# Immortal-ibr/Verifiable-Federated-Training-with-Zero-Knowledge-Proofs-ZK-FL-

Hardware: AMD Instinct MI355X
Metric: Groth16 proofs/sec (training-step circuit, ~2^18 constraints) at 1/8 MI355X (higher is better)
Workload: dtype u32; 1 GPU; groth16 prove, sgd_verified(128, 4, 7, 1000) (BATCH,DIM,DEPTH,PRECISION); constraints=261399, wires=262810, domain=262144, global_batch=20, step=20 proofs per GPU (one per slot), parallelism=replicas1, slots_in_flight=20, hw_queues=28

## Files before the change

### include/zkfl.h

```cpp
#ifndef ZKFL_H
#define ZKFL_H

#include <stddef.h>
#include <stdint.h>

#ifdef __cplusplus
extern "C" {
#endif

#define ZKFL_OK 0
#define ZKFL_E_ARG -1
#define ZKFL_E_FORMAT -2
#define ZKFL_E_PRIME -3
#define ZKFL_E_MISMATCH -4
#define ZKFL_E_DEVICE -5
#define ZKFL_E_OOM -6
#define ZKFL_E_CONSTRAINT -7
#define ZKFL_E_KEY -8

typedef struct zkfl_ctx zkfl_ctx;
typedef struct zkfl_key zkfl_key;
typedef struct zkfl_witness zkfl_witness;
typedef struct zkfl_wprog zkfl_wprog;
typedef struct zkfl_vkey zkfl_vkey;

int zkfl_version(void);
const char* zkfl_build_id(void);
const char* zkfl_last_error(void);
int zkfl_device_count(int* count);

int zkfl_ctx_create(int device, zkfl_ctx** out);
int zkfl_ctx_destroy(zkfl_ctx* ctx);
int zkfl_ctx_set_profiling(zkfl_ctx* ctx, int enabled);
int zkfl_ctx_profile(zkfl_ctx* ctx, const char* name, double* total_ms, uint64_t* launches, double* units,
                     double* median_ms);
int zkfl_ctx_profile_reset(zkfl_ctx* ctx);
int zkfl_ctx_synchronize(zkfl_ctx* ctx);

int zkfl_zkey_load(zkfl_ctx* ctx, const uint8_t* buf, size_t len, zkfl_key** out);
typedef struct zkfl_zkey_file zkfl_zkey_file;
int zkfl_zkey_file_open(const char* path, zkfl_zkey_file** out);
int zkfl_zkey_load_file(zkfl_ctx* ctx, const zkfl_zkey_file* f, zkfl_key** out);
int zkfl_zkey_file_close(zkfl_zkey_file* f);
int zkfl_key_free(zkfl_key* key);
int zkfl_key_info(const zkfl_key* key, uint32_t* n_vars, uint32_t* n_public, uint32_t* domain_size);
int zkfl_key_ab_shared(const zkfl_key* key, uint32_t* d_form, uint32_t* shared_wires, uint32_t* a_bases);
int zkfl_debug_ab_partition(const uint8_t* sec_a, const uint8_t* sec_b1, size_t n, uint32_t shard, uint32_t n_shards,
                            uint32_t* counts, uint32_t* sidx_out, uint8_t* img_out);
typedef struct zkfl_groups_info {
  uint32_t grouped;
  uint32_t learned;
  uint32_t groups;
  uint32_t non_rep;
  uint32_t bases[4];
  uint32_t bases_rep[4];
  uint32_t builds;
  uint32_t last_miss;
  double build_ms;
} zkfl_groups_info;
int zkfl_key_set_groups(zkfl_key* key, const uint32_t* rep, size_t n_vars);
int zkfl_key_learn_groups(zkfl_ctx* ctx, zkfl_key* key, const zkfl_witness* w);
int zkfl_key_groups(const zkfl_key* key, zkfl_groups_info* out);
int zkfl_debug_groups(const uint8_t* values, const uint8_t* sig, size_t n, uint32_t* rep_out, const uint32_t* sidx,
                      size_t n_bases, uint32_t u_base, uint32_t* sidx_out, uint32_t* start_out,
                      uint32_t* members_out);
int zkfl_key_set_slots(zkfl_key* key, int slots);

int zkfl_groth16_prove(zkfl_ctx* ctx, zkfl_key* key, const uint8_t* wtns, size_t wtns_len,
                       const uint8_t* rs, uint8_t proof_out[256], uint8_t* pub_out, size_t* npub);

int zkfl_witness_upload(zkfl_ctx* ctx, const zkfl_key* key, const uint8_t* wtns, size_t wtns_len,
                        zkfl_witness** out);
int zkfl_witness_free(zkfl_witness* w);
int zkfl_groth16_prove_resident(zkfl_ctx* ctx, zkfl_key* key, const zkfl_witness* w, const uint8_t* rs,
                                uint8_t proof_out[256]);
int zkfl_groth16_prove_batch(zkfl_ctx* ctx, zkfl_key* key, size_t n, const zkfl_witness* const* w,
                             const uint8_t* rs, uint8_t* proofs_out);

int zkfl_groth16_prove_multi(zkfl_ctx* ctx, size_t n, zkfl_key* const* keys, const zkfl_witness* const* w,
                             const uint8_t* rs, uint8_t* proofs_out);

int zkfl_zkey_load_shard(zkfl_ctx* ctx, const uint8_t* buf, size_t len, uint32_t shard, uint32_t n_shards,
                         zkfl_key** out);
int zkfl_key_shard(const zkfl_key* key, uint32_t* shard, uint32_t* n_shards);
int zkfl_groth16_prove_part_batch(zkfl_ctx* ctx, zkfl_key* key, size_t n, const zkfl_witness* const* w,
                                  const uint8_t* rs, uint8_t* parts_out);
int zkfl_groth16_assemble(zkfl_ctx* ctx, size_t n, size_t n_parts, const uint8_t* parts, const uint8_t* rs,
                          uint8_t* proofs_out);

int zkfl_debug_prove_parts(zkfl_ctx* ctx, zkfl_key* key, const uint8_t* wtns, size_t wtns_len, uint8_t* h_out,
                           uint8_t* msm_out);

int zkfl_debug_glv_split(const uint8_t k[32], uint8_t out[40]);

int zkfl_debug_g1_glv_mul(zkfl_ctx* ctx, size_t n, const uint8_t* points, const uint8_t* scalars, uint8_t* out);

int zkfl_debug_wtrace(zkfl_ctx* ctx, int op, uint32_t cap, void* out, uint32_t* count);

int zkfl_debug_ntt_coset(zkfl_ctx* ctx, uint8_t* data, uint32_t logn, uint32_t nvec, size_t vstride, int col_max);

int zkfl_msm_g1(zkfl_ctx* ctx, const uint8_t* bases, const uint8_t* scalars, size_t n, uint8_t out[64]);
int zkfl_msm_g2(zkfl_ctx* ctx, const uint8_t* bases, const uint8_t* scalars, size_t n, uint8_t out[128]);
int zkfl_ntt_coset(zkfl_ctx* ctx, uint8_t* data, uint32_t logn);

int zkfl_wprog_load(zkfl_ctx* ctx, const uint8_t* prog, size_t len, zkfl_wprog** out);
int zkfl_wprog_free(zkfl_wprog* prog);
int zkfl_wprog_info(const zkfl_wprog* prog, uint32_t* n_wires, uint32_t* n_inputs, uint32_t* n_public);
size_t zkfl_wtns_size(const zkfl_wprog* prog);
int zkfl_wprog_parse_inputs(const uint8_t* prog, size_t len, const char* input_json, uint8_t* inputs_out, size_t cap,
                            size_t* n_inputs);
int zkfl_witness_compute_json(zkfl_ctx* ctx, const zkfl_wprog* prog, const char* input_json, uint8_t* wtns_out);
int zkfl_witness_compute(zkfl_ctx* ctx, const zkfl_wprog* prog, size_t n, const uint8_t* inputs, uint8_t* wtns_out);
int zkfl_witness_compute_resident(zkfl_ctx* ctx, const zkfl_wprog* prog, const zkfl_key* key, size_t n,
                                  const uint8_t* inputs, zkfl_witness** out);

int zkfl_groth16_full_prove_batch(zkfl_ctx* ctx, zkfl_key* key, const zkfl_wprog* prog, size_t n,
                                  const uint8_t* inputs, const uint8_t* rs, uint8_t* proofs_out, uint8_t* pubs_out);

int zkfl_groth16_full_prove_json(zkfl_ctx* ctx, zkfl_key* key, const zkfl_wprog* prog, const char* input_json,
                                 const uint8_t* rs, uint8_t proof_out[256], uint8_t* pub_out);

int zkfl_groth16_full_prove_json_batch(zkfl_ctx* ctx, zkfl_key* key, const zkfl_wprog* prog, size_t n,
                                       const char* const* input_jsons, const uint8_t* rs, uint8_t* proofs_out,
                                       uint8_t* pubs_out);

int zkfl_groth16_full_prove_multi(zkfl_ctx* ctx, size_t n, zkfl_key* const* keys, const zkfl_wprog* const* progs,
                                  const uint8_t* const* inputs, const uint8_t* rs, uint8_t* proofs_out,
                                  uint8_t* const* pubs_out);

typedef struct zkfl_r1cs zkfl_r1cs;
typedef struct {
  uint32_t n_wires, n_pub_out, n_pub_in, n_prv_in, n_constraints;
  uint64_t n_labels, n_terms;
} zkfl_r1cs_header;
typedef struct {
  uint32_t n_failed, first;
  uint8_t a[32], b[32], c[32];
} zkfl_r1cs_report;
int zkfl_r1cs_parse(const uint8_t* buf, size_t len, zkfl_r1cs_header* out);
int zkfl_r1cs_load(zkfl_ctx* ctx, const uint8_t* buf, size_t len, zkfl_r1cs** out);
int zkfl_r1cs_info(const zkfl_r1cs* r1cs, zkfl_r1cs_header* out);
int zkfl_r1cs_free(zkfl_r1cs* r1cs);
int zkfl_r1cs_check(zkfl_ctx* ctx, const zkfl_r1cs* r1cs, size_t n, const uint8_t* const* wtns, const size_t* wtns_len,
                    zkfl_r1cs_report* reports);
int zkfl_r1cs_check_resident(zkfl_ctx* ctx, const zkfl_r1cs* r1cs, size_t n, const zkfl_witness* const* w,
                             zkfl_r1cs_report* reports);

#define ZKFL_KEYCHECK_HEADER 0
#define ZKFL_KEYCHECK_POINTS 1
#define ZKFL_KEYCHECK_COEFFICIENTS 2
#define ZKFL_KEYCHECK_A 3
#define ZKFL_KEYCHECK_B1 4
#define ZKFL_KEYCHECK_B2 5
#define ZKFL_KEYCHECK_IC 6
#define ZKFL_KEYCHECK_C 7
#define ZKFL_KEYCHECK_H 8
#define ZKFL_KEYCHECK_N 9
#define ZKFL_KEYCHECK_PASS 0
#define ZKFL_KEYCHECK_FAIL 1
#define ZKFL_KEYCHECK_NOT_RUN 2
typedef struct {
  uint32_t power;
  const uint8_t *L, *L2, *La, *Lb, *H0;
  size_t L_len, L2_len, La_len, Lb_len, H0_len;
  const uint8_t *alpha1, *beta1, *beta2;
} zkfl_ptau_view;
typedef struct {
  uint32_t status[ZKFL_KEYCHECK_N];
  uint32_t point_section, point_index, point_count;
  uint32_t coef_matrix, coef_row, coef_count;
} zkfl_zkey_report;
int zkfl_zkey_check(zkfl_ctx* ctx, const zkfl_r1cs* r1cs, const uint8_t* zkey, size_t zkey_len,
                    const zkfl_ptau_view* ptau, const uint8_t* rho, const uint8_t* sigma, zkfl_zkey_report* report);

int zkfl_groth16_verify(zkfl_ctx* ctx, const uint8_t* vk, size_t vk_len, const uint8_t* pub, size_t npub,
                        const uint8_t proof[256]);
int zkfl_groth16_verify_batch(zkfl_ctx* ctx, const uint8_t* vk, size_t vk_len, size_t n, const uint8_t* pubs,
                              size_t npub, const uint8_t* proofs, int32_t* results);
int zkfl_pairing(zkfl_ctx* ctx, size_t n, const uint8_t* g1, const uint8_t* g2, uint8_t* gt_out);
int zkfl_debug_miller_loop(zkfl_ctx* ctx, size_t n, const uint8_t* g1, const uint8_t* g2, uint8_t* out);

#define ZKFL_VERIFY_WAVE_MAX_PUBLIC 32
int zkfl_vkey_load(zkfl_ctx* ctx, const uint8_t* vk, size_t vk_len, zkfl_vkey** out);
int zkfl_vkey_info(const zkfl_vkey* key, uint32_t* n_public);
int zkfl_vkey_free(zkfl_vkey* key);

#define ZKFL_VERIFY_AUTO 0
#define ZKFL_VERIFY_LANES 1
#define ZKFL_VERIFY_WAVES 2
#define ZKFL_VERIFY_AUTO_WAVES_MAX 4096
int zkfl_groth16_verify_multi(zkfl_ctx* ctx, size_t n, const zkfl_vkey* const* vkeys, const uint8_t* const* pubs,
                              const size_t* npubs, const uint8_t* proofs, int32_t* results, int schedule);
typedef struct {
  uint32_t keys;
  uint32_t screened;
  uint32_t combined;
  uint32_t passed;
  uint32_t fallback;
} zkfl_round_report;
int zkfl_groth16_verify_round(zkfl_ctx* ctx, size_t n, const zkfl_vkey* const* vkeys, const uint8_t* const* pubs,
                              const size_t* npubs, const uint8_t* proofs, const uint8_t* z, int32_t* results,
                              zkfl_round_report* report);
int zkfl_debug_verify_round(zkfl_ctx* ctx, size_t n, const zkfl_vkey* const* vkeys, const uint8_t* const* pubs,
                            const size_t* npubs, const uint8_t* proofs, const uint8_t* z, size_t chunk,
                            uint8_t gt_out[384], int32_t* screened_out);
int zkfl_debug_wave_pairing(zkfl_ctx* ctx, size_t n, const uint8_t* g1, const uint8_t* g2, int final_exp,
                            uint8_t* out);

int zkfl_poseidon_params(uint32_t t, uint8_t* consts_out, uint8_t* xy_out, uint32_t* rp_out);
int zkfl_poseidon_batch(zkfl_ctx* ctx, uint32_t arity, size_t n, const uint8_t* inputs, uint8_t* out);
int zkfl_vector_hash_batch(zkfl_ctx* ctx, uint32_t len, size_t n, const uint8_t* values, uint8_t* out);
#define ZKFL_MERKLE_MAX_DEPTH 30
int zkfl_merkle_build(zkfl_ctx* ctx, const uint8_t* leaves, size_t n, uint32_t depth, uint8_t* tree_out);
int zkfl_dataset_commit(zkfl_ctx* ctx, const uint8_t* values, size_t n, uint32_t len, uint32_t depth,
                        uint8_t* tree_out);

int zkfl_setup_g1_gen_mul(zkfl_ctx* ctx, const uint8_t* scalars, size_t n, uint8_t* out);
int zkfl_setup_g2_gen_mul(zkfl_ctx* ctx, const uint8_t* scalars, size_t n, uint8_t* out);
// ... 15 lines not shown
```

### verifiable-federated-training-with-zero-knowledge-proofs-zk-fl-_amd/csrc/groups.h

```cpp
#pragma once
#include <stddef.h>
#include <stdint.h>
#include <string.h>

#include <algorithm>
#include <unordered_map>
#include <vector>

namespace zkfl {

inline bool groups_valid(const uint32_t* rep, size_t n) {
  for (size_t i = 0; i < n; i++)
    if (rep[i] > i || rep[rep[i]] != rep[i]) return false;
  return true;
}

inline void groups_learn(const uint32_t* w, size_t n, std::vector<uint32_t>& rep) {
  rep.resize(n);
  std::vector<uint32_t> big;
  for (size_t i = 0; i < n; i++) {
    rep[i] = (uint32_t)i;
    const uint32_t* v = w + 8 * i;
    if (v[4] | v[5] | v[6] | v[7]) big.push_back((uint32_t)i);
  }
  std::sort(big.begin(), big.end(), [&](uint32_t a, uint32_t b) {
    const int c = memcmp(w + 8 * (size_t)a, w + 8 * (size_t)b, 32);
    return c ? c < 0 : a < b;
  });
  for (size_t k = 1; k < big.size(); k++)
    if (memcmp(w + 8 * (size_t)big[k], w + 8 * (size_t)big[k - 1], 32) == 0) rep[big[k]] = rep[big[k - 1]];
}

inline void groups_refine(uint32_t* rep, const uint8_t* sig, size_t n) {
  std::unordered_map<uint64_t, uint32_t> first;
  for (size_t i = 0; i < n; i++) {
    const uint32_t r = rep[i];
    if ((sig[i] & ~sig[r]) == 0) continue;
    rep[i] = first.emplace((uint64_t)r << 8 | sig[i], (uint32_t)i).first->second;
  }
}

struct GroupQuery {
  std::vector<uint32_t> sidx;
  std::vector<uint32_t> start;
  std::vector<uint32_t> members;
  uint32_t groups = 0;
  uint32_t non_rep = 0;
};

inline void groups_query(const uint32_t* rep, uint32_t n_vars, const uint32_t* sidx, size_t n, uint32_t u_base,
                         GroupQuery& q) {
  constexpr uint32_t NONE = 0xFFFFFFFFu;
  std::vector<uint32_t> slot_of(n_vars, NONE), to(n, NONE);
  for (size_t j = 0; j < n; j++)
    if (sidx[j] < n_vars) slot_of[sidx[j]] = (uint32_t)j;
  q.sidx.assign(sidx, sidx + n);
  q.start.assign(n + 1, 0);
  q.groups = q.non_rep = 0;
  for (size_t j = 0; j < n; j++) {
    const uint32_t i = sidx[j];
    if (i >= n_vars || rep[i] == i || slot_of[rep[i]] == NONE) continue;
    to[j] = slot_of[rep[i]];
    q.sidx[j] = u_base + i;
    if (q.start[to[j] + 1]++ == 0) q.groups++;
    q.non_rep++;
  }
  for (size_t j = 0; j < n; j++) q.start[j + 1] += q.start[j];
  q.members.resize(q.non_rep);
  std::vector<uint32_t> cur(q.start.begin(), q.start.end() - 1);
  for (size_t j = 0; j < n; j++)
    if (to[j] != NONE) q.members[cur[to[j]]++] = (uint32_t)j;
}

}

#ifdef __HIPCC__
#include <hip/hip_runtime.h>

#include "curve.h"

namespace zkfl {

template <class F>
void group_sums(hipStream_t st, const Affine<F>* bases_w, int W, size_t n, const uint32_t* start,
                const uint32_t* members, Affine<F>* out);
void group_delta(hipStream_t st, const Fr* w, const uint32_t* rep, uint32_t n, Fr* u, uint32_t* cnt,
                 uint32_t* miss_out);

}
#endif
```

### verifiable-federated-training-with-zero-knowledge-proofs-zk-fl-_amd/csrc/groups.hip

```cpp
#include <hip/hip_runtime.h>
#include <stdint.h>

#include <chrono>
#include <cstdio>
#include <vector>

#include "devbufs.h"
#include "groups.h"
#include "objects.h"

using namespace zkfl;

namespace {

ZK_DEV Fq from_m29(const Fq& a) {
  Fq c = fp_zero<FqP>();
  c.v[7] = 0x08000000u;
  return fp_mul(a, c);
}

template <class F>
ZK_DEV Affine<F> load_base(const Affine<F>* __restrict__ p) {
  Affine<F> a = *p;
  Fq* q = reinterpret_cast<Fq*>(&a);
#pragma unroll
  for (int k = 0; k < (int)(sizeof(Affine<F>) / sizeof(Fq)); k++) q[k] = from_m29(q[k]);
  return a;
}

template <class F>
__global__ void __launch_bounds__(64) k_group_sums(const Affine<F>* __restrict__ bases_w, int W, size_t n,
                                                   const uint32_t* __restrict__ start,
                                                   const uint32_t* __restrict__ members, Affine<F>* __restrict__ out) {
  const size_t j = (size_t)blockIdx.x * blockDim.x + threadIdx.x;
  if (j >= n) return;
  const Affine<F> p = load_base<F>(bases_w + j * W);
  const uint32_t b = start[j], e = start[j + 1];
  if (b == e) {
    out[j] = p;
    return;
  }
  XYZZ<F> acc = xyzz_from_affine<F>(p);
  for (uint32_t m = b; m < e; m++) acc = xyzz_madd<F>(acc, load_base<F>(bases_w + (size_t)members[m] * W));
  out[j] = xyzz_to_affine<F>(acc);
}

constexpr int DELTA_T = 256;

__global__ void __launch_bounds__(DELTA_T) k_group_delta(const Fr* __restrict__ w, const uint32_t* __restrict__ rep,
                                                         uint32_t n, Fr* __restrict__ u, uint32_t* __restrict__ cnt,
                                                         uint32_t* __restrict__ miss_out) {
  ZK_LIGHT();
  const uint32_t i = blockIdx.x * DELTA_T + threadIdx.x;
  int nz = 0;
  if (i < n) {
    const uint32_t r = rep[i];
    Fr v = fp_zero<FrP>();
    if (r != i) {
      v = fp_sub(w[i], w[r]);
#pragma unroll
      for (int k = 0; k < 8; k++) nz |= v.v[k] != 0;
    }
    u[i] = v;
  }
  const int blk = __syncthreads_count(nz);
  if (threadIdx.x == 0) {
    if (blk) atomicAdd(&cnt[0], (uint32_t)blk);
    __threadfence();
    if (atomicAdd(&cnt[1], 1u) == gridDim.x - 1) {
      __threadfence();
      *miss_out = atomicExch(&cnt[0], 0u);
      cnt[1] = 0;
    }
  }
}

}

namespace zkfl {

template <class F>
void group_sums(hipStream_t st, const Affine<F>* bases_w, int W, size_t n, const uint32_t* start,
                const uint32_t* members, Affine<F>* out) {
  if (n) hipLaunchKernelGGL(k_group_sums<F>, dim3(zk_grid(n, 64)), dim3(64), 0, st, bases_w, W, n, start, members, out);
}
template void group_sums<FqOps>(hipStream_t, const G1Aff*, int, size_t, const uint32_t*, const uint32_t*, G1Aff*);
template void group_sums<Fq2Ops>(hipStream_t, const G2Aff*, int, size_t, const uint32_t*, const uint32_t*, G2Aff*);

void group_delta(hipStream_t st, const Fr* w, const uint32_t* rep, uint32_t n, Fr* u, uint32_t* cnt,
                 uint32_t* miss_out) {
  hipLaunchKernelGGL(k_group_delta, dim3(zk_grid(n, DELTA_T)), dim3(DELTA_T), 0, st, w, rep, n, u, cnt, miss_out);
}

void key_groups_release(zkfl_key* k) {
  msm_bases_free(k->gA);
  msm_bases_free(k->gB1);
  msm_bases_free(k->gB2);
  msm_bases_free(k->gCH);
  if (k->grp.d_rep) (void)hipFree(k->grp.d_rep);
  const uint32_t builds = k->grp.builds;
  k->grp = KeyGroups();
  k->grp.builds = builds;
}

}

namespace {

template <class F>
hipError_t build_query(const MsmBases<F>& plain, MsmBases<F>& out, const GroupQuery& q, uint32_t extra_start,
                       DevBufs& D, hipStream_t st) {
  ZK_CHECK(msm_bases_alloc(out, plain.n, plain.c));
  if (plain.n == 0) return hipSuccess;
  uint32_t *d_start, *d_members;
  Affine<F>* d_img;
  ZK_CHECK(D.get(&d_start, q.start.size()));
  ZK_CHECK(D.get(&d_members, q.members.size()));
  ZK_CHECK(D.get(&d_img, plain.n));
  ZK_CHECK(hipMemcpyAsync(d_start, q.start.data(), q.start.size() * 4, hipMemcpyHostToDevice, st));
  if (!q.members.empty())
    ZK_CHECK(hipMemcpyAsync(d_members, q.members.data(), q.members.size() * 4, hipMemcpyHostToDevice, st));
  group_sums<F>(st, plain.bases_w, msm_w_of(plain.c), plain.n, d_start, d_members, d_img);
  ZK_CHECK(hipGetLastError());
  return msm_bases_set(out, d_img, q.sidx.data(), extra_start, st, false);
}

int key_build_groups(zkfl_key* k, std::vector<uint32_t>& rep, bool learned, double host_ms) {
  const auto t0 = std::chrono::steady_clock::now();
  HIP_TRY(hipSetDevice(k->ctx->device), "hipSetDevice");
  int rc = key_reset_graphs(k);
  if (rc) return rc;
  key_groups_release(k);
  const uint32_t nV = k->nVars, X = nV, dom = k->n;
  std::vector<uint8_t> sig(nV, 0);
  for (int qi = 0; qi < 4; qi++)
    for (uint32_t i : k->q_sidx[qi])
      if (i < nV) sig[i] |= (uint8_t)(1u << qi);
  groups_refine(rep.data(), sig.data(), nV);
  const uint32_t u_base[4] = {X + 4, X + 4, X + 4, X + dom + 4};
  GroupQuery q[4];
  for (int qi = 0; qi < 4; qi++)
    groups_query(rep.data(), nV, k->q_sidx[qi].data(), k->q_sidx[qi].size(), u_base[qi], q[qi]);
  hipStream_t st = k->ctx->st;
  hipError_t e;
  {
    DevBufs D;
    e = hipMalloc(&k->grp.d_rep, (size_t)(nV ? nV : 1) * 4);
    if (e == hipSuccess) e = hipMemcpyAsync(k->grp.d_rep, rep.data(), (size_t)nV * 4, hipMemcpyHostToDevice, st);
    if (e == hipSuccess) e = build_query(k->bA, k->gA, q[0], X, D, st);
    if (e == hipSuccess) e = build_query(k->bB1, k->gB1, q[1], X, D, st);
    if (e == hipSuccess) e = build_query(k->bB2, k->gB2, q[2], X, D, st);
    if (e == hipSuccess) e = build_query(k->bCH, k->gCH, q[3], X, D, st);
    const hipError_t es = hipStreamSynchronize(st);
    if (e == hipSuccess) e = es;
  }
  if (e != hipSuccess) {
    key_groups_release(k);
    return hip_fail(e, "grouped base sets");
  }
  KeyGroups& g = k->grp;
  g.on = true;
  g.learned = learned;
  for (uint32_t i = 0; i < nV; i++) g.non_rep += rep[i] != i;
  std::vector<uint8_t> has(nV, 0);
  for (uint32_t i = 0; i < nV; i++)
    if (rep[i] != i && !has[rep[i]]) {
      has[rep[i]] = 1;
      g.groups++;
    }
  for (int qi = 0; qi < 4; qi++) {
    g.bases[qi] = (uint32_t)k->q_sidx[qi].size();
    g.bases_rep[qi] = g.bases[qi] - q[qi].non_rep;
  }
  g.builds++;
  g.build_ms = host_ms + std::chrono::duration<double, std::milli>(std::chrono::steady_clock::now() - t0).count();
  fprintf(stderr,
          "zkfl: key of %u wires: %u groups, %u non-representative wires; bases A %u -> %u, B %u -> %u, C+H %u -> %u; "
          "%s and built in %.1f ms\n",
          nV, g.groups, g.non_rep, g.bases[0], g.bases_rep[0], g.bases[1], g.bases_rep[1], g.bases[3], g.bases_rep[3],
          learned ? "learned" : "set", g.build_ms);
  return ZKFL_OK;
}

int groups_allowed(const zkfl_key* k) {
  if (k->nshards != 1) return fail(ZKFL_E_ARG, "groups: a sharded key keeps the plain form");
  if (!k->ctx->opts.groups) return fail(ZKFL_E_ARG, "groups: turned off on this context (ZKFL_GROUPS=0)");
  return ZKFL_OK;
}

}

int zkfl::key_learn_groups(zkfl_ctx* ctx, zkfl_key* k, const Fr* d_w) {
  const auto t0 = std::chrono::steady_clock::now();
  HIP_TRY(hipSetDevice(ctx->device), "hipSetDevice");
  std::vector<uint32_t> w((size_t)k->nVars * 8), rep;
  HIP_TRY(hipMemcpy(w.data(), d_w, w.size() * 4, hipMemcpyDeviceToHost), "download witness");
  groups_learn(w.data(), k->nVars, rep);
  const double ms = std::chrono::duration<double, std::milli>(std::chrono::steady_clock::now() - t0).count();
  return key_build_groups(k, rep, true, ms);
}

extern "C" {

int zkfl_key_set_groups(zkfl_key* key, const uint32_t* rep, size_t n_vars) {
  if (!key) return fail(ZKFL_E_ARG, "null key");
  if (!rep) {
    HIP_TRY(hipSetDevice(key->ctx->device), "hipSetDevice");
    const int rc = key_reset_graphs(key);
    if (rc) return rc;
    key_groups_release(key);
    return ZKFL_OK;
  }
  int rc = groups_allowed(key);
  if (rc) return rc;
  if (n_vars != key->nVars) return fail(ZKFL_E_ARG, "groups: rep must hold one entry per wire of the key");
  if (!groups_valid(rep, n_vars)) return fail(ZKFL_E_ARG, "groups: rep[i] <= i and rep[rep[i]] == rep[i] must hold");
  std::vector<uint32_t> r(rep, rep + n_vars);
  return key_build_groups(key, r, false, 0.0);
}

int zkfl_key_learn_groups(zkfl_ctx* ctx, zkfl_key* key, const zkfl_witness* w) {
  if (!ctx || !key || !w) return fail(ZKFL_E_ARG, "null argument");
  if (key->ctx != ctx) return fail(ZKFL_E_ARG, "groups: key of another context");
  if (w->key != key) return fail(ZKFL_E_MISMATCH, "witness uploaded for another key");
  const int rc = groups_allowed(key);
  if (rc) return rc;
  return key_learn_groups(ctx, key, w->d);
}

int zkfl_key_groups(const zkfl_key* key, zkfl_groups_info* out) {
  if (!key || !out) return fail(ZKFL_E_ARG, "null argument");
  const KeyGroups& g = key->grp;
  *out = zkfl_groups_info();
  out->grouped = g.on;
  out->learned = g.learned;
  out->groups = g.groups;
  out->non_rep = g.non_rep;
  for (int i = 0; i < 4; i++) {
    out->bases[i] = g.on ? g.bases[i] : (uint32_t)key->q_sidx[i].size();
    out->bases_rep[i] = g.on ? g.bases_rep[i] : out->bases[i];
  }
  out->builds = g.builds;
  out->last_miss = g.last_miss;
  out->build_ms = g.build_ms;
  return ZKFL_OK;
}

int zkfl_debug_groups(const uint8_t* values, const uint8_t* sig, size_t n, uint32_t* rep_out, const uint32_t* sidx,
                      size_t n_bases, uint32_t u_base, uint32_t* sidx_out, uint32_t* start_out,
                      uint32_t* members_out) {
  if (!rep_out || n > 0x7FFFFFF0u || (n_bases && !sidx)) return fail(ZKFL_E_ARG, "debug_groups: bad arguments");
  std::vector<uint32_t> rep;
  if (values) {
    std::vector<uint32_t> w(n * 8);
    memcpy(w.data(), values, n * 32);
    groups_learn(w.data(), n, rep);
  } else {
    rep.assign(rep_out, rep_out + n);
    if (!groups_valid(rep.data(), n)) return fail(ZKFL_E_ARG, "debug_groups: not a partition");
  }
  if (sig) groups_refine(rep.data(), sig, n);
  memcpy(rep_out, rep.data(), n * 4);
  if (sidx_out || start_out || members_out) {
    GroupQuery q;
    groups_query(rep.data(), (uint32_t)n, sidx, n_bases, u_base, q);
    if (sidx_out) memcpy(sidx_out, q.sidx.data(), n_bases * 4);
    if (start_out) memcpy(start_out, q.start.data(), (n_bases + 1) * 4);
    if (members_out && !q.members.empty()) memcpy(members_out, q.members.data(), q.members.size() * 4);
  }
  return ZKFL_OK;
}

}
```

### verifiable-federated-training-with-zero-knowledge-proofs-zk-fl-_amd/csrc/objects.h

```cpp
#pragma once
#include <hip/hip_runtime.h>
#include <stdint.h>

#include <atomic>
#include <string>
#include <vector>

#include "curve.h"
#include "field.h"
#include "msm_api.h"
#include "ntt.h"
#include "prof.h"
#include "wtrace.h"
#include "zkfl.h"

namespace zkfl {
struct VkDev;
struct PosTables;
struct WProg;

int fail(int code, const std::string& msg);
int hip_fail(hipError_t e, const char* where);
}

#define HIP_TRY(x, where)                              \
  do {                                                 \
    hipError_t _e = (x);                               \
    if (_e != hipSuccess) return ::zkfl::hip_fail(_e, where); \
  } while (0)

using namespace zkfl;

struct WitPipe;

struct SchedOpts {
  bool graph = true;
  bool stagger = true;
  bool lowlat = true;
  bool fast_wsum = true;
  int small_logn = 16;
  bool ab_shared = true;
  bool groups = true;
  int group_min_batch = 8;
};

struct zkfl_ctx {
  int device = 0;
  hipStream_t st = nullptr;
  SchedOpts opts;
  Profiler prof;
  zkfl::VkDev* vk = nullptr;
  zkfl::PosTables* pos = nullptr;
  void* asm_buf = nullptr;
  size_t asm_cap = 0;
  WtBuf wt;
  std::atomic<int> refs{1};
};

struct ProofSlot {
  hipStream_t st_main = nullptr;
  hipEvent_t ev_done = nullptr;
  MsmScratch<FqOps> g1s;
#if ZK_KNOCKOUT & 2
  MsmScratch<FqOps> g1s_ko[3];
#endif
  MsmTail<FqOps> g1t[4];
  MsmScratch<Fq2Ops> g2s;
  MsmTail<Fq2Ops> g2t;
  Fr* extra = nullptr;
  Fr* abc = nullptr;
  Fr* abc_head = nullptr;
  Fr* abc_tail = nullptr;
  Fr* h = nullptr;
  uint32_t* grp_cnt = nullptr;
  zkfl_key* key = nullptr;
  bool grouped_run = false;
  G1P* res = nullptr;
  G2P* resB2 = nullptr;
  Fr* d_rs = nullptr;
  uint32_t* d_parts = nullptr;
  uint8_t* pinned = nullptr;
  hipStream_t st_lat[2] = {nullptr, nullptr};
  hipEvent_t ev_lat[3] = {nullptr, nullptr, nullptr};
  MsmScratch<FqOps> g1s_b;
  MsmScratch<FqOps> g1s_a;
  hipGraph_t graph = nullptr;
  hipGraphExec_t graph_exec = nullptr;
  Fr* w_stage = nullptr;
  uint32_t direct_proofs = 0;
  bool nnz_alias = false;
  bool busy = false;
  int index = 0;
  size_t job = 0;
  uint8_t* out_proof = nullptr;
  uint8_t* out_part = nullptr;
};

struct KeyGroups {
  bool on = false;
  bool learned = false;
  uint32_t groups = 0;
  uint32_t non_rep = 0;
  uint32_t bases[4] = {0, 0, 0, 0};
  uint32_t bases_rep[4] = {0, 0, 0, 0};
  double build_ms = 0;
  uint32_t builds = 0;
  uint32_t last_miss = 0;
  uint32_t* d_rep = nullptr;
};

struct zkfl_key {
  zkfl_ctx* ctx = nullptr;
  uint32_t nVars = 0, nPub = 0, n = 0;
  int logn = 0;
  size_t nC = 0;
  size_t K = 0;
  uint32_t* rows = nullptr;
  uint32_t* cols = nullptr;
  Fr* coefs = nullptr;
  uint32_t cshift = 0;
  MsmBases<FqOps> bA, bB1;
  MsmBases<Fq2Ops> bB2;
  MsmBases<FqOps> bCH;
  MsmBases<FqOps> gA, gB1, gCH;
  MsmBases<Fq2Ops> gB2;
  KeyGroups grp;
  std::vector<uint32_t> q_sidx[4];
  Fr* dbg_zero = nullptr;
  bool a_diff = false;
  uint32_t ab_shared = 0;
  bool share_b = false;
  bool front = false;
  int msm_c = MSM_C;
  NttPlan ntt;
  std::vector<ProofSlot*> slots;
  int max_slots = 3;
  uint32_t shard = 0, nshards = 1;
  WitPipe* wpipe = nullptr;
};

struct zkfl_witness {
  const zkfl_key* key = nullptr;
  Fr* d = nullptr;
  std::vector<uint8_t> pub;
};

struct zkfl_wprog {
  zkfl_ctx* ctx = nullptr;
  zkfl::WProg* p = nullptr;
};

struct zkfl_vkey {
  zkfl_ctx* ctx = nullptr;
  zkfl::VkDev* vk = nullptr;
  void* wtab = nullptr;
  bool wave_ok = false;
};

namespace zkfl {
void ctx_retain(zkfl_ctx* ctx);
void ctx_release(zkfl_ctx* ctx);
int get_slot(zkfl_key* k, size_t idx, ProofSlot** out);
void key_release_slots(zkfl_key* k);
int key_reset_graphs(zkfl_key* k);
void key_groups_release(zkfl_key* k);
int key_learn_groups(zkfl_ctx* ctx, zkfl_key* k, const Fr* d_w);
constexpr size_t MISS_OFF = 456;
}
```

### verifiable-federated-training-with-zero-knowledge-proofs-zk-fl-_amd/csrc/poly.h

```cpp
#pragma once
#include <hip/hip_runtime.h>
#include <stdint.h>

#include "field.h"
#include "glv.h"

namespace zkfl {

constexpr uint32_t ABC_L = 16;

struct AbcTerms {
  const uint32_t* cols;
  const Fr* coefs;
  uint32_t cshift;
};

struct ProofStart {
  uint4* buckets[5];
  uint32_t nvec[5];
  uint32_t* nnz[5];
  uint32_t* live[5];
  int n;
  const uint64_t* w_src_host;
  uint4* w_dst;
  uint32_t w_nvec;
};

constexpr int RS_WORDS = (64 + 4 * (int)sizeof(GlvScalar)) / 4;

__device__ __forceinline__ Fr abc_row(const uint32_t* __restrict__ rp, uint32_t r, uint32_t K,
                                      const Fr* __restrict__ head, const Fr* __restrict__ tail,
                                      const Fr* __restrict__ abc) {
  const uint32_t s = rp[r], e = rp[r + 1];
  if (s == e) return fp_zero<FrP>();
  const uint32_t c0 = s / ABC_L, c1 = (e - 1) / ABC_L;
  const bool starts = (s == c0 * ABC_L);
  if (c0 == c1) {
    const uint32_t cend = (c0 + 1) * ABC_L < K ? (c0 + 1) * ABC_L : K;
    if (starts) return head[c0];
    if (e == cend) return tail[c0];
    return abc[r];
  }
  Fr acc = starts ? head[c0] : tail[c0];
  for (uint32_t c = c0 + 1; c <= c1; c++) acc = fp_add(acc, head[c]);
  return acc;
}

void abc_chunks(hipStream_t st, const uint32_t* rp, uint32_t nrows, const AbcTerms& T, const Fr* w, uint32_t K,
                Fr* head, Fr* tail, Fr* abc);
void abc_rows(hipStream_t st, const uint32_t* rp, size_t n, uint32_t K, const Fr* head, const Fr* tail, Fr* abc);
void join_h(hipStream_t st, const Fr* abc, size_t n, Fr* h);
void proof_start(hipStream_t st, const uint32_t* rs_host, uint32_t* d_rs, Fr* extra, int plain, uint32_t* res3,
                 const ProofStart& ps);
void fr_std_to_mont(hipStream_t st, Fr* a, size_t n);
void fr_mont_to_std(hipStream_t st, Fr* a, size_t n);

}
```

### verifiable-federated-training-with-zero-knowledge-proofs-zk-fl-_amd/csrc/poly.hip

```cpp
#include "poly.h"

#include "common.h"
#include "msm_api.h"
#include "wtrace.h"

using namespace zkfl;

namespace {

template <bool PACKED>
__global__ void __launch_bounds__(64) k_abc_chunks(const uint32_t* __restrict__ rp, uint32_t nrows, AbcTerms T,
                                                   const Fr* __restrict__ w, uint32_t K, Fr* __restrict__ head,
                                                   Fr* __restrict__ tail, Fr* __restrict__ abc) {
  ZK_WT(WT_ABC);
  ZK_LIGHT();
  const uint32_t c = blockIdx.x * blockDim.x + threadIdx.x;
  const uint32_t p0 = c * ABC_L;
  if (p0 >= K) return;
  const uint32_t p1 = p0 + ABC_L < K ? p0 + ABC_L : K;
  const uint32_t* __restrict__ cols = T.cols;
  const Fr* __restrict__ coefs = T.coefs;
  const uint32_t cmask = PACKED ? (1u << T.cshift) - 1u : 0xFFFFFFFFu;
  auto coef_of = [&](uint32_t t, uint32_t p) { return PACKED ? coefs[t >> T.cshift] : coefs[p]; };
  auto row_of = [&](uint32_t p, uint32_t lo) {
    uint32_t hi = nrows - 1;
    while (lo < hi) {
      const uint32_t mid = (lo + hi + 1) >> 1;
      if (rp[mid] <= p) lo = mid;
      else hi = mid - 1;
    }
    return lo;
  };
  uint32_t r = row_of(p0, 0), rend = rp[r + 1];
  Fr acc = fp_zero<FrP>();
  bool first = true;
  uint32_t t1 = (p0 + 1 < p1) ? cols[p0 + 1] : 0u;
  const uint32_t t0 = cols[p0];
  Fr wv = w[t0 & cmask], cf = coef_of(t0, p0);
  for (uint32_t p = p0; p < p1; p++) {
    Fr wn, cn;
    uint32_t t2 = 0;
    if (p + 1 < p1) {
      wn = w[t1 & cmask];
      cn = coef_of(t1, p + 1);
    }
    if (p + 2 < p1) t2 = cols[p + 2];
    if (p == rend) {
      if (first) head[c] = acc;
      else abc[r] = acc;
      first = false;
      acc = fp_zero<FrP>();
      r++;
      rend = rp[r + 1];
      if (rend == p) {
        r = row_of(p, r);
        rend = rp[r + 1];
      }
    }
    acc = fp_add(acc, fp_mul(cf, wv));
    wv = wn;
    cf = cn;
    t1 = t2;
  }
  if (first) head[c] = acc;
  else tail[c] = acc;
}

__global__ void __launch_bounds__(256) k_abc_rows(const uint32_t* __restrict__ rp, size_t n, uint32_t K,
                                                  const Fr* __restrict__ head, const Fr* __restrict__ tail,
                                                  Fr* __restrict__ abc) {
  ZK_WT(WT_ABC_ROWS);
  ZK_LIGHT();
  const size_t j = (size_t)blockIdx.x * blockDim.x + threadIdx.x;
  if (j >= n) return;
  const Fr a = abc_row(rp, (uint32_t)j, K, head, tail, abc);
  const Fr b = abc_row(rp, (uint32_t)(n + j), K, head, tail, abc);
  abc[j] = a;
  abc[n + j] = b;
  abc[2 * n + j] = fp_mul(a, b);
}

__global__ void k_join(const Fr* __restrict__ abc, size_t n, Fr* __restrict__ h) {
  ZK_WT(WT_JOIN);
  ZK_LIGHT();
  size_t j = (size_t)blockIdx.x * blockDim.x + threadIdx.x;
  if (j >= n) return;
#if ZK_KNOCKOUT & 4
  Fr v = fp_add(fp_mul(abc[j], abc[n + j]), abc[2 * n + j]);
#else
  Fr v = fp_sub(fp_mul(abc[j], abc[n + j]), abc[2 * n + j]);
#endif
  h[j] = fp_from_mont(v);
}

__global__ void __launch_bounds__(256) k_proof_start(const uint32_t* __restrict__ rs_host, uint32_t* __restrict__ d_rs,
                                                     Fr* __restrict__ extra, int plain, uint32_t* __restrict__ res3,
                                                     const ProofStart ps) {
  ZK_WT(WT_SET_EXTRA);
  ZK_LIGHT();
  const int y = blockIdx.y;
  if (ps.w_dst) {
    __shared__ const uint4* src;
    if (threadIdx.x == 0) src = reinterpret_cast<const uint4*>(*ps.w_src_host);
    __syncthreads();
    const size_t nb = (size_t)gridDim.x * gridDim.y * blockDim.x;
    for (size_t i = ((size_t)y * gridDim.x + blockIdx.x) * blockDim.x + threadIdx.x; i < ps.w_nvec; i += nb)
      ps.w_dst[i] = src[i];
  }
  if (y == 0 && blockIdx.x == 2 && threadIdx.x < RS_WORDS) d_rs[threadIdx.x] = rs_host[threadIdx.x];
  if (y == 0 && blockIdx.x == 0 && threadIdx.x == 0) {
    const Fr* rs = reinterpret_cast<const Fr*>(rs_host);
    Fr one = fp_zero<FrP>();
    one.v[0] = plain ? 0u : 1u;
    Fr r = plain ? fp_zero<FrP>() : rs[0];
    Fr s = plain ? fp_zero<FrP>() : rs[1];
    extra[0] = one;
    extra[1] = r;
    extra[2] = s;
    extra[3] = fp_from_mont(fp_neg(fp_mul(fp_to_mont(r), fp_to_mont(s))));
  }
  if (y == 0 && blockIdx.x == 1 && res3 && threadIdx.x < sizeof(G1P) / 4) res3[threadIdx.x] = 0u;
  if (y >= ps.n) return;
  uint4* b = ps.buckets[y];
  const size_t nv = ps.nvec[y];
  for (size_t i = (size_t)blockIdx.x * blockDim.x + threadIdx.x; i < nv; i += (size_t)gridDim.x * blockDim.x)
    b[i] = make_uint4(0, 0, 0, 0);
  if (blockIdx.x == 0 && threadIdx.x == 0) *ps.nnz[y] = 0;
  if (blockIdx.x == 0 && threadIdx.x < MSM_LIVE_LEVELS) ps.live[y][threadIdx.x] = 0;
}

__global__ void k_fr_std_to_mont(Fr* __restrict__ a, size_t n) {
  size_t i = (size_t)blockIdx.x * blockDim.x + threadIdx.x;
  if (i >= n) return;
  a[i] = fp_to_mont(a[i]);
}

__global__ void k_fr_mont_to_std(Fr* __restrict__ a, size_t n) {
  size_t i = (size_t)blockIdx.x * blockDim.x + threadIdx.x;
  if (i >= n) return;
  a[i] = fp_from_mont(a[i]);
}

}

namespace zkfl {

hipError_t zk_wtrace_bind_poly(const WtBuf& b) { return zk_wtrace_bind_tu(b); }

void abc_chunks(hipStream_t st, const uint32_t* rp, uint32_t nrows, const AbcTerms& T, const Fr* w, uint32_t K,
                Fr* head, Fr* tail, Fr* abc) {
  if (T.cshift)
    hipLaunchKernelGGL(k_abc_chunks<true>, dim3(zk_grid((K + ABC_L - 1) / ABC_L, 64)), dim3(64), 0, st, rp, nrows, T, w,
                       K, head, tail, abc);
  else
    hipLaunchKernelGGL(k_abc_chunks<false>, dim3(zk_grid((K + ABC_L - 1) / ABC_L, 64)), dim3(64), 0, st, rp, nrows, T, w,
                       K, head, tail, abc);
}

void abc_rows(hipStream_t st, const uint32_t* rp, size_t n, uint32_t K, const Fr* head, const Fr* tail, Fr* abc) {
  hipLaunchKernelGGL(k_abc_rows, dim3(zk_grid(n, 256)), dim3(256), 0, st, rp, n, K, head, tail, abc);
}

void join_h(hipStream_t st, const Fr* abc, size_t n, Fr* h) {
  hipLaunchKernelGGL(k_join, dim3(zk_grid(n, 256)), dim3(256), 0, st, abc, n, h);
}

void proof_start(hipStream_t st, const uint32_t* rs_host, uint32_t* d_rs, Fr* extra, int plain, uint32_t* res3,
                 const ProofStart& ps) {
  hipLaunchKernelGGL(k_proof_start, dim3(128, ps.n), dim3(256), 0, st, rs_host, d_rs, extra, plain, res3, ps);
}

void fr_std_to_mont(hipStream_t st, Fr* a, size_t n) {
  hipLaunchKernelGGL(k_fr_std_to_mont, dim3(zk_grid(n, 256)), dim3(256), 0, st, a, n);
}

void fr_mont_to_std(hipStream_t st, Fr* a, size_t n) {
  hipLaunchKernelGGL(k_fr_mont_to_std, dim3(zk_grid(n, 256)), dim3(256), 0, st, a, n);
}

}
```

### verifiable-federated-training-with-zero-knowledge-proofs-zk-fl-_amd/csrc/prove.hip

```cpp
#include <hip/hip_runtime.h>
#include <stdint.h>
#include <string.h>
#include <sys/random.h>

#include <algorithm>
#include <atomic>
#include <chrono>
#include <condition_variable>
#include <mutex>
#include <string>
#include <thread>
#include <vector>

#include "assemble.h"
#include "glv.h"
#include "groups.h"
#include "host_parse.h"
#include "objects.h"
#include "poly.h"
#include "witness.h"

using namespace zkfl;

namespace {

constexpr size_t W_PTR_OFF = 448;

inline uint32_t* proof_out(ProofSlot* s) { return reinterpret_cast<uint32_t*>(s->pinned); }

void slot_drop_lowlat(ProofSlot* s) {
  for (hipStream_t& st : s->st_lat)
    if (st) {
      (void)hipStreamSynchronize(st);
      (void)hipStreamDestroy(st);
      st = nullptr;
    }
  for (hipEvent_t& e : s->ev_lat)
    if (e) {
      (void)hipEventDestroy(e);
      e = nullptr;
    }
}

void slot_release(ProofSlot* s) {
  if (!s) return;
  if (s->st_main) (void)hipStreamSynchronize(s->st_main);
  slot_drop_lowlat(s);
  if (s->nnz_alias) s->g2t.nnz = nullptr;
  msm_scratch_free(s->g1s);
#if ZK_KNOCKOUT & 2
  for (MsmScratch<FqOps>& x : s->g1s_ko) msm_scratch_free(x);
#endif
  for (auto& t : s->g1t) msm_tail_free(t);
  msm_scratch_free(s->g2s);
  msm_tail_free(s->g2t);
  void* ptrs[] = {s->abc, s->abc_head, s->abc_tail, s->h, s->res, s->resB2, s->d_rs, s->d_parts,
                  s->w_stage, s->grp_cnt};
  for (void* p : ptrs)
    if (p) (void)hipFree(p);
  if (s->pinned) (void)hipHostFree(s->pinned);
  msm_scratch_free(s->g1s_b);
  msm_scratch_free(s->g1s_a);
  if (s->graph_exec) (void)hipGraphExecDestroy(s->graph_exec);
  if (s->graph) (void)hipGraphDestroy(s->graph);
  if (s->ev_done) (void)hipEventDestroy(s->ev_done);
  if (s->st_main) (void)hipStreamDestroy(s->st_main);
  delete s;
}

hipError_t slot_side_resources(ProofSlot* s, const zkfl_key* k, bool need_streams) {
  if (need_streams) {
    for (hipStream_t& st : s->st_lat)
      if (!st) ZK_CHECK(hipStreamCreateWithFlags(&st, hipStreamNonBlocking));
    for (hipEvent_t& e : s->ev_lat)
      if (!e) ZK_CHECK(hipEventCreateWithFlags(&e, hipEventDisableTiming));
  }
  if (!s->g1s_a.keys_out) ZK_CHECK(msm_scratch_alloc(s->g1s_a, k->bA.n, k->msm_c, k->ctx->st));
  if (!s->g1s_b.keys_out) ZK_CHECK(msm_scratch_alloc(s->g1s_b, k->bB1.n, k->msm_c, k->ctx->st));
  return hipSuccess;
}

hipError_t slot_create(zkfl_key* k, ProofSlot** out) {
  ProofSlot* s = new ProofSlot();
  *out = s;
  const size_t nV = k->nVars, n = k->n;
  const size_t cap1 = std::max<size_t>({k->bA.n, k->bB1.n, k->bCH.n});
  hipStream_t st = k->ctx->st;
  ZK_CHECK(hipStreamCreateWithFlags(&s->st_main, hipStreamNonBlocking));
  ZK_CHECK(hipEventCreateWithFlags(&s->ev_done, hipEventDisableTiming));
  const int c = k->msm_c;
  ZK_CHECK(msm_scratch_alloc(s->g1s, cap1, c, st));
#if ZK_KNOCKOUT & 2
  for (MsmScratch<FqOps>& x : s->g1s_ko) {
    ZK_CHECK(msm_scratch_alloc(x, cap1, c, st));
    ZK_CHECK(hipMemsetAsync(x.keys_out, 0, cap1 * msm_w_of(c) * sizeof(uint16_t), st));
    ZK_CHECK(hipMemsetAsync(x.vals_out, 0, cap1 * msm_w_of(c) * sizeof(uint32_t), st));
  }
#endif
  const size_t caps[4] = {k->bA.n, k->bB1.n, k->bCH.n, k->bCH.n};
  for (int i = 0; i < 4; i++) ZK_CHECK(msm_tail_alloc(s->g1t[i], caps[i], c));
  ZK_CHECK(msm_scratch_alloc(s->g2s, k->bB2.n, c, st));
  ZK_CHECK(msm_tail_alloc(s->g2t, k->bB2.n, c));
  if (k->share_b && !ZK_KNOCKOUT) {
    ZK_CHECK(hipFree(s->g2t.nnz));
    s->g2t.nnz = s->g1t[1].nnz;
    s->nnz_alias = true;
  }
  if (k->ctx->opts.graph) ZK_CHECK(hipMalloc(&s->w_stage, nV * 32));
  if (k->front) ZK_CHECK(slot_side_resources(s, k, false));
  const bool may_group = k->ctx->opts.groups && k->nshards == 1;
  ZK_CHECK(hipMalloc(&s->h, (n + 4 + (may_group ? nV : 0)) * 32));
  s->extra = s->h + n;
  ZK_CHECK(hipMalloc(&s->grp_cnt, 2 * sizeof(uint32_t)));
  ZK_CHECK(hipMemsetAsync(s->grp_cnt, 0, 2 * sizeof(uint32_t), st));
  s->key = k;
  ZK_CHECK(hipMalloc(&s->abc, n * 3 * 32));
  const size_t abc_chunks = (k->K + ABC_L - 1) / ABC_L + 1;
  ZK_CHECK(hipMalloc(&s->abc_head, abc_chunks * 32));
  ZK_CHECK(hipMalloc(&s->abc_tail, abc_chunks * 32));
  ZK_CHECK(hipMalloc(&s->res, 5 * sizeof(G1P)));
  ZK_CHECK(hipMalloc(&s->resB2, sizeof(G2P)));
  ZK_CHECK(hipMalloc(&s->d_rs, 2 * 32 + 4 * sizeof(GlvScalar)));
  ZK_CHECK(hipMalloc(&s->d_parts, PART_WORDS * 4));
  ZK_CHECK(hipHostMalloc(&s->pinned, 2048, hipHostMallocCoherent));
  return hipStreamSynchronize(st);
}

}

int zkfl::get_slot(zkfl_key* k, size_t idx, ProofSlot** out) {
  size_t want = idx % (size_t)k->max_slots;
  while (k->slots.size() <= want) {
    ProofSlot* s = nullptr;
    hipError_t e = slot_create(k, &s);
    if (e != hipSuccess) {
      slot_release(s);
      return hip_fail(e, "proof slot allocation");
    }
    s->index = (int)k->slots.size();
    k->slots.push_back(s);
  }
  *out = k->slots[want];
  return ZKFL_OK;
}

constexpr int WIT_SETS = 4;
struct WitPipe {
  struct Set {
    Fr* W = nullptr;
    Fr* d = nullptr;
    uint32_t* in = nullptr;
    uint32_t* fail = nullptr;
    Fr** outs = nullptr;
    uint8_t* pin_in = nullptr;
    hipEvent_t ev = nullptr;
  };
  size_t G = 0, nw = 0, n_in = 0;
  hipStream_t st = nullptr;
  Set set[WIT_SETS];
};

namespace {

void wpipe_release(WitPipe* p) {
  if (!p) return;
  if (p->st) (void)hipStreamSynchronize(p->st);
  for (auto& b : p->set) {
    for (void* q : {(void*)b.W, (void*)b.d, (void*)b.in, (void*)b.fail, (void*)b.outs})
      if (q) (void)hipFree(q);
    if (b.pin_in) (void)hipHostFree(b.pin_in);
    if (b.ev) (void)hipEventDestroy(b.ev);
  }
  if (p->st) (void)hipStreamDestroy(p->st);
  delete p;
}

}

int zkfl::key_reset_graphs(zkfl_key* k) {
  for (ProofSlot* s : k->slots)
    if (s->busy) return fail(ZKFL_E_ARG, "slots busy");
  for (ProofSlot* s : k->slots) {
    if (s->st_main) (void)hipStreamSynchronize(s->st_main);
    if (s->graph_exec) (void)hipGraphExecDestroy(s->graph_exec);
    if (s->graph) (void)hipGraphDestroy(s->graph);
    s->graph_exec = nullptr;
    s->graph = nullptr;
  }
  return ZKFL_OK;
}

void zkfl::key_release_slots(zkfl_key* k) {
  wpipe_release(k->wpipe);
  k->wpipe = nullptr;
  for (ProofSlot* s : k->slots) slot_release(s);
  k->slots.clear();
}

namespace {

hipError_t wpipe_get(zkfl_key* k, size_t G, size_t nw, size_t n_in, WitPipe** out) {
  WitPipe* p = k->wpipe;
  if (p && p->G == G && p->nw == nw && p->n_in == n_in) {
    *out = p;
    return hipSuccess;
  }
  wpipe_release(p);
  k->wpipe = p = new WitPipe();
  p->G = G;
  p->nw = nw;
  p->n_in = n_in;
  ZK_CHECK(hipStreamCreateWithFlags(&p->st, hipStreamNonBlocking));
  for (auto& b : p->set) {
    ZK_CHECK(hipMalloc(&b.W, G * nw * 32));
    ZK_CHECK(hipMalloc(&b.d, G * nw * 32));
    ZK_CHECK(hipMalloc(&b.in, G * n_in * 32 + 16));
    ZK_CHECK(hipMalloc(&b.fail, G * 4));
    ZK_CHECK(hipMalloc(&b.outs, G * sizeof(Fr*)));
    ZK_CHECK(hipHostMalloc(&b.pin_in, G * n_in * 32 + 16));
    ZK_CHECK(hipEventCreateWithFlags(&b.ev, hipEventDisableTiming));
    std::vector<Fr*> ptrs(G);
    for (size_t j = 0; j < G; j++) ptrs[j] = b.d + j * nw;
    ZK_CHECK(hipMemcpy(b.outs, ptrs.data(), G * sizeof(Fr*), hipMemcpyHostToDevice));
  }
  *out = p;
  return hipSuccess;
}

int get_rs(const uint8_t* rs, uint32_t out[16]) {
  if (rs) {
    memcpy(out, rs, 64);
    if (!fr_lt_r(out) || !fr_lt_r(out + 8)) return fail(ZKFL_E_ARG, "r/s must be < r");
    return ZKFL_OK;
  }
  for (int k = 0; k < 2; k++) {
    for (int tries = 0;; tries++) {
      uint8_t b[32];
      if (getrandom(b, 32, 0) != 32) return fail(ZKFL_E_DEVICE, "getrandom failed");
      b[31] &= 0x3f;
      memcpy(out + 8 * k, b, 32);
      if (fr_lt_r(out + 8 * k)) break;
      if (tries > 64) return fail(ZKFL_E_DEVICE, "rng");
    }
  }
  return ZKFL_OK;
}

enum class ProofMode {
  Proof,
  Parts,
  SplitPart,
};

enum class Schedule { Lowlat, Front, Chain };

struct ProofPlan {
  ProofMode mode;
  Schedule schedule;
  bool share_b_sort;
  bool light_first;
  bool joint_tails;
  bool fast_wsum;
  bool graph;
  bool grouped;
};

struct PlanBases {
  const MsmBases<FqOps>&A, &B1, &CH;
  const MsmBases<Fq2Ops>& B2;
};
inline PlanBases plan_bases(const zkfl_key* k, const ProofPlan& p) {
  if (p.grouped) return {k->gA, k->gB1, k->gCH, k->gB2};
  return {k->bA, k->bB1, k->bCH, k->bB2};
}

ProofPlan plan_proof(const SchedOpts& o, const zkfl_key* k, const ProofSlot* s, ProofMode mode, bool batch_of_one,
                     const Profiler* prof) {
  ProofPlan p = {};
  p.mode = mode;
  p.grouped = mode == ProofMode::Proof && k->grp.on && !ZK_KNOCKOUT;
  const bool plain = mode == ProofMode::Proof && k->share_b && !prof->serialize && !ZK_KNOCKOUT;
  const bool want_lowlat = batch_of_one && o.lowlat;
  p.graph = o.graph && s->w_stage && !want_lowlat && plain && !prof->on && s->direct_proofs > 0;
  p.share_b_sort = k->share_b && !(ZK_KNOCKOUT & 32);
  if (want_lowlat && plain) {
    p.schedule = Schedule::Lowlat;
    p.fast_wsum = o.fast_wsum;
    return p;
  }
  p.joint_tails = p.share_b_sort && k->front;
  const bool front = p.joint_tails && mode != ProofMode::Parts && !(ZK_KNOCKOUT & 2);
  p.schedule = front ? Schedule::Front : Schedule::Chain;
  p.light_first = !front && o.stagger && (s->index & 1) && !prof->serialize;
  p.fast_wsum = o.fast_wsum && k->logn <= o.small_logn;
  return p;
}

inline const GlvScalar* glv_halves(const ProofSlot* s) {
  return reinterpret_cast<const GlvScalar*>(reinterpret_cast<const uint8_t*>(s->d_rs) + 64);
}

void start(zkfl_key* k, ProofSlot* s, const ProofPlan& p) {
  const bool parts = p.mode == ProofMode::Parts;
  const int ntails = parts ? 4 : 3;
  ProofStart ps = {};
  auto add = [&](void* buckets, size_t bytes, uint32_t* nnz, uint32_t* live) {
    ps.buckets[ps.n] = static_cast<uint4*>(buckets);
    ps.nvec[ps.n] = (uint32_t)(bytes / sizeof(uint4));
    ps.nnz[ps.n] = nnz;
    ps.live[ps.n] = live;
    ps.n++;
  };
  const size_t nb = msm_nb_of(k->msm_c);
  for (int i = 0; i < ntails; i++) add(s->g1t[i].buckets, nb * sizeof(G1P), s->g1t[i].nnz, s->g1t[i].live);
  if (p.share_b_sort) add(s->g2t.buckets, nb * sizeof(G2P), s->g2t.nnz, s->g2t.live);
  uint32_t* res3 = parts ? nullptr : reinterpret_cast<uint32_t*>(s->res + 3);
  if (p.graph) {
    ps.w_src_host = reinterpret_cast<const uint64_t*>(s->pinned + W_PTR_OFF);
    ps.w_dst = reinterpret_cast<uint4*>(s->w_stage);
    ps.w_nvec = (uint32_t)((size_t)k->nVars * 32 / sizeof(uint4));
  }
  proof_start(s->st_main, reinterpret_cast<const uint32_t*>(s->pinned + 256), reinterpret_cast<uint32_t*>(s->d_rs),
              s->extra, parts, res3, ps);
}

hipError_t abc_ntt(zkfl_key* k, ProofSlot* s, const Fr* d_w, hipStream_t st, Profiler* prof) {
  const size_t n = k->n;
  int pi = prof->begin("abc", st);
  if (k->K) {
    const uint32_t K = (uint32_t)k->K;
    const AbcTerms T = {k->cols, k->coefs, k->cshift};
    abc_chunks(st, k->rows, (uint32_t)(2 * n), T, d_w, K, s->abc_head, s->abc_tail, s->abc);
  }
  abc_rows(st, k->rows, n, (uint32_t)k->K, s->abc_head, s->abc_tail, s->abc);
  prof->end(pi, st, (double)k->K);
  pi = prof->begin("ntt", st);
  if (!(ZK_KNOCKOUT & 4)) ZK_CHECK(ntt_coset_shift(k->ntt, s->abc, 3, n, st));
  prof->end(pi, st, 3.0 * (double)n);
  join_h(st, s->abc, n, s->h);
  return hipSuccess;
}

hipError_t b2_from_b1_sort(const MsmBases<Fq2Ops>& bB2, ProofSlot* s, const MsmScratch<FqOps>& sorted, hipStream_t st,
                           Profiler* prof) {
  if (!s->nnz_alias)
    ZK_CHECK(hipMemcpyAsync(s->g2t.nnz, s->g1t[1].nnz, sizeof(uint32_t), hipMemcpyDeviceToDevice, st));
  return msm_accumulate_sorted(bB2, sorted.keys_out, sorted.vals_out, s->g2t, st, prof, "msm_accumulate_g2");
}

int finish(const zkfl_key* k, ProofSlot* s, const ProofPlan& p, Profiler* prof) {
  hipStream_t st = s->st_main;
  if (k->a_diff) fold_a(st, s->res);
  if (p.mode == ProofMode::SplitPart) {
    part_out(st, s->res, s->resB2, s->d_parts);
    HIP_TRY(hipMemcpyAsync(s->pinned + 512, s->d_parts, PART_WORDS * 4, hipMemcpyDeviceToHost, st), "download part");
  }
  if (p.mode == ProofMode::Proof && !(ZK_KNOCKOUT & 1)) {
    const int pa = prof->begin("assemble", st);
    assemble(st, 1, s->res, s->resB2, glv_halves(s), proof_out(s));
    prof->end(pa, st, 1.0);
  }
  return ZKFL_OK;
}

int run_lowlat(zkfl_key* k, ProofSlot* s, const Fr* d_w, const ProofPlan& p, Profiler* prof) {
  HIP_TRY(slot_side_resources(s, k, true), "latency schedule resources");
  hipStream_t st = s->st_main, sb = s->st_lat[0], sa = s->st_lat[1];
  hipEvent_t ev = s->ev_lat[0], ev_b2 = s->ev_lat[1], ev_t = s->ev_lat[2];
  const uint32_t *W = (const uint32_t*)d_w, *E = (const uint32_t*)s->extra;
  const PlanBases b = plan_bases(k, p);
  MsmTail<FqOps>* tails[3] = {&s->g1t[0], &s->g1t[1], &s->g1t[2]};
  G1P* outs[3] = {s->res + 0, s->res + 1, s->res + 2};
  MsmTail<Fq2Ops>* t2 = &s->g2t;
  G2P* o2 = s->resB2;
  HIP_TRY(hipEventRecord(ev, st), "event");
  HIP_TRY(hipStreamWaitEvent(sb, ev, 0), "wait");
  HIP_TRY(msm_sort(b.B1, s->g1s_b, s->g1t[1].nnz, W, E, sb), "msm B sort");
  HIP_TRY(hipEventRecord(ev, sb), "event");
  HIP_TRY(hipStreamWaitEvent(sa, ev, 0), "wait");
  HIP_TRY(b2_from_b1_sort(b.B2, s, s->g1s_b, sb, prof), "msm B2");
  HIP_TRY(msm_tails(&t2, &o2, 1, sb, p.fast_wsum), "msm B2 tail");
  HIP_TRY(hipEventRecord(ev_b2, sb), "event");
  HIP_TRY(msm_accumulate_sorted(b.B1, s->g1s_b.keys_out, s->g1s_b.vals_out, s->g1t[1], sa, prof,
                                   "msm_accumulate_g1"), "msm B1");
  HIP_TRY(msm_accumulate(b.A, s->g1s_a, s->g1t[0], W, E, sa, prof, "msm_accumulate_g1"), "msm A");
  HIP_TRY(msm_tails(tails, outs, 2, sa, p.fast_wsum), "msm tails A, B1");
  if (k->a_diff) fold_a(sa, s->res);
  assemble_t(sa, s->res, glv_halves(s), proof_out(s));
  HIP_TRY(hipEventRecord(ev_t, sa), "event");
  HIP_TRY(abc_ntt(k, s, d_w, st, prof), "ntt");
  HIP_TRY(msm_accumulate(b.CH, s->g1s, s->g1t[2], W, (const uint32_t*)s->h, st, prof, "msm_accumulate_g1"),
          "msm C+H");
  HIP_TRY(msm_tails(&tails[2], &outs[2], 1, st, p.fast_wsum), "msm tail C+H");
  HIP_TRY(hipStreamWaitEvent(st, ev_b2, 0), "wait");
  HIP_TRY(hipStreamWaitEvent(st, ev_t, 0), "wait");
  const int pa = prof->begin("assemble", st);
  assemble_c(st, s->res, s->resB2, proof_out(s));
  prof->end(pa, st, 1.0);
  return ZKFL_OK;
}

int run_front(zkfl_key* k, ProofSlot* s, const Fr* d_w, const ProofPlan& p, Profiler* prof) {
  hipStream_t st = s->st_main;
  const uint32_t *W = (const uint32_t*)d_w, *E = (const uint32_t*)s->extra;
  HIP_TRY(abc_ntt(k, s, d_w, st, prof), "ntt");
  const PlanBases b = plan_bases(k, p);
  const MsmBases<FqOps>* bs[3] = {&b.A, &b.B1, &b.CH};
  MsmScratch<FqOps>* ss[3] = {&s->g1s_a, &s->g1s_b, &s->g1s};
  MsmTail<FqOps>* tails[3] = {&s->g1t[0], &s->g1t[1], &s->g1t[2]};
  uint32_t* nn[3] = {s->g1t[0].nnz, s->g1t[1].nnz, s->g1t[2].nnz};
  const uint32_t* sc[3] = {W, W, W};
  const uint32_t* ex[3] = {E, E, (const uint32_t*)s->h};
  HIP_TRY(msm_sort_multi(bs, ss, nn, sc, ex, 3, st), "msm A, B1, C+H sorts");
  const uint16_t* kk[3] = {ss[0]->keys_out, ss[1]->keys_out, ss[2]->keys_out};
  const uint32_t* vv[3] = {ss[0]->vals_out, ss[1]->vals_out, ss[2]->vals_out};
  HIP_TRY(msm_accumulate_sorted_multi(bs, kk, vv, tails, 3, st), "msm A, B1, C+H");
  HIP_TRY(b2_from_b1_sort(b.B2, s, s->g1s_b, st, prof), "msm B2");
  G1P* outs[3] = {s->res + 0, s->res + 1, s->res + 2};
  MsmTail<Fq2Ops>* t2 = &s->g2t;
  G2P* o2 = s->resB2;
  HIP_TRY(msm_tails_joint(tails, outs, 3, &t2, &o2, 1, st, p.fast_wsum), "msm tails (G1 + G2)");
  return finish(k, s, p, prof);
}

int run_chain(zkfl_key* k, ProofSlot* s, const Fr* d_w, const ProofPlan& p, Profiler* prof) {
  hipStream_t st = s->st_main;
  const bool parts = p.mode == ProofMode::Parts;
  if (parts && !k->dbg_zero) return fail(ZKFL_E_ARG, "parity hook: zeros not allocated");
  const uint32_t *W = (const uint32_t*)d_w, *E = (const uint32_t*)s->extra, *H = (const uint32_t*)s->h,
                 *Z = (const uint32_t*)k->dbg_zero;
#if ZK_KNOCKOUT & 2
  MsmScratch<FqOps>&sA = s->g1s_ko[0], &sB = s->g1s_ko[1], &sCH = s->g1s_ko[2];
#else
  MsmScratch<FqOps>&sA = s->g1s, &sB = s->g1s, &sCH = s->g1s;
#endif
  const PlanBases b = plan_bases(k, p);
  MsmTail<FqOps>* tails[4] = {&s->g1t[0], &s->g1t[1], &s->g1t[2], &s->g1t[3]};
  G1P* outs[4] = {s->res + 0, s->res + 1, s->res + 2, s->res + 3};
  MsmTail<Fq2Ops>* t2 = &s->g2t;
  G2P* o2 = s->resB2;
  if (!p.share_b_sort && !(ZK_KNOCKOUT & 32))
    HIP_TRY(msm_run(b.B2, s->g2s, s->g2t, W, E, s->resB2, st, prof, "msm_accumulate_g2"), "msm B2");
  if (p.light_first) HIP_TRY(abc_ntt(k, s, d_w, st, prof), "ntt");
  HIP_TRY(msm_accumulate(b.A, sA, s->g1t[0], W, E, st, prof, "msm_accumulate_g1"), "msm A");
  if (p.share_b_sort) {
    HIP_TRY(msm_sort(b.B1, sB, s->g1t[1].nnz, W, E, st), "msm B1 sort");
    HIP_TRY(msm_accumulate_sorted(b.B1, sB.keys_out, sB.vals_out, s->g1t[1], st, prof, "msm_accumulate_g1"),
            "msm B1");
    HIP_TRY(b2_from_b1_sort(b.B2, s, sB, st, prof), "msm B2");
    if (!p.joint_tails) HIP_TRY(msm_tails(&t2, &o2, 1, st, p.fast_wsum), "msm B2 tail");
  } else {
    HIP_TRY(msm_accumulate(b.B1, sB, s->g1t[1], W, E, st, prof, "msm_accumulate_g1"), "msm B1");
  }
  if (parts) HIP_TRY(msm_accumulate(b.CH, s->g1s, s->g1t[2], W, Z, st, prof, "msm_accumulate_g1"), "msm C");
  if (!p.light_first) HIP_TRY(abc_ntt(k, s, d_w, st, prof), "ntt");
  if (parts)
    HIP_TRY(msm_accumulate(b.CH, s->g1s, s->g1t[3], Z, H, st, prof, "msm_accumulate_g1"), "msm H");
  else
    HIP_TRY(msm_accumulate(b.CH, sCH, s->g1t[2], W, H, st, prof, "msm_accumulate_g1"), "msm C+H");
  const int ntails = parts ? 4 : 3;
  if (p.joint_tails)
    HIP_TRY(msm_tails_joint(tails, outs, ntails, &t2, &o2, 1, st, p.fast_wsum), "msm tails (G1 + G2)");
  else
    HIP_TRY(msm_tails(tails, outs, ntails, st, p.fast_wsum), "msm tails");
  return finish(k, s, p, prof);
}

int run_proof(zkfl_ctx* ctx, zkfl_key* k, ProofSlot* s, const Fr* d_w, const ProofPlan& p) {
  Profiler* prof = &ctx->prof;
  const int pp = prof->begin("prove", s->st_main);
  start(k, s, p);
  if (p.grouped)
    group_delta(s->st_main, d_w, k->grp.d_rep, k->nVars, s->extra + 4, s->grp_cnt,
                reinterpret_cast<uint32_t*>(s->pinned + MISS_OFF));
  const int rc = p.schedule == Schedule::Lowlat  ? run_lowlat(k, s, d_w, p, prof)
                 : p.schedule == Schedule::Front ? run_front(k, s, d_w, p, prof)
                                                 : run_chain(k, s, d_w, p, prof);
  if (rc) return rc;
  prof->end(pp, s->st_main, 1.0);
  return ZKFL_OK;
}

int enqueue_proof_graph(zkfl_ctx* ctx, zkfl_key* k, ProofSlot* s, const ProofPlan& p) {
  hipStream_t st = s->st_main;
  if (!s->graph_exec) {
    HIP_TRY(hipStreamBeginCapture(st, hipStreamCaptureModeThreadLocal), "begin capture");
    const int rc = run_proof(ctx, k, s, s->w_stage, p);
    hipError_t e = hipStreamEndCapture(st, &s->graph);
    if (rc == ZKFL_OK && e == hipSuccess) e = hipGraphInstantiate(&s->graph_exec, s->graph, nullptr, nullptr, 0);
    if (rc || e != hipSuccess) {
      if (s->graph) (void)hipGraphDestroy(s->graph);
      s->graph = nullptr;
      s->graph_exec = nullptr;
      return rc ? rc : hip_fail(e, "graph capture");
    }
  }
  HIP_TRY(hipGraphLaunch(s->graph_exec, st), "graph launch");
  return ZKFL_OK;
}

int enqueue_proof(zkfl_ctx* ctx, zkfl_key* k, ProofSlot* s, const Fr* d_w, const uint32_t rs_host[16], ProofMode mode,
                  bool batch_of_one) {
  memcpy(s->pinned + 256, rs_host, 64);
  GlvScalar* ks = reinterpret_cast<GlvScalar*>(s->pinned + 320);
  glv_split(rs_host + 8, ks[0], ks[1]);
  glv_split(rs_host, ks[2], ks[3]);
  const ProofPlan p = plan_proof(ctx->opts, k, s, mode, batch_of_one, &ctx->prof);
  s->grouped_run = p.grouped;
  int rc;
  if (p.graph) {
    const uint64_t src = reinterpret_cast<uint64_t>(d_w);
    memcpy(s->pinned + W_PTR_OFF, &src, sizeof(src));
    rc = enqueue_proof_graph(ctx, k, s, p);
  } else {
    s->direct_proofs++;
    rc = run_proof(ctx, k, s, d_w, p);
  }
  if (rc) return rc;
  HIP_TRY(hipEventRecord(s->ev_done, s->st_main), "event");
  HIP_TRY(hipGetLastError(), "launch");
  return ZKFL_OK;
}

constexpr int WAIT_US = 50;
static hipError_t host_wait(hipEvent_t ev, bool poll) {
  if (!poll) return hipEventSynchronize(ev);
  for (;;) {
    const hipError_t e = hipEventQuery(ev);
    if (e != hipErrorNotReady) return e;
    std::this_thread::sleep_for(std::chrono::microseconds(WAIT_US));
  }
}

int wait_slot(ProofSlot* s, bool poll = false) {
  HIP_TRY(host_wait(s->ev_done, poll), "sync");
  if (s->out_proof) memcpy(s->out_proof, s->pinned, 256);
  if (s->out_part) memcpy(s->out_part, s->pinned + 512, PART_WORDS * 4);
  if (s->grouped_run) memcpy(&s->key->grp.last_miss, s->pinned + MISS_OFF, 4);
  s->grouped_run = false;
  s->busy = false;
  return ZKFL_OK;
}

struct Job {
  zkfl_key* key = nullptr;
  const Fr* w = nullptr;
  hipEvent_t w_ready = nullptr;
  const uint8_t* rs = nullptr;
  uint8_t* proof_out = nullptr;
  uint8_t* part_out = nullptr;
};

int learn_for_batch(zkfl_ctx* ctx, const Job& J, size_t n) {
  zkfl_key* k = J.key;
  if (!ctx->opts.groups || ZK_KNOCKOUT || n < (size_t)ctx->opts.group_min_batch || k->nshards != 1 || J.part_out)
    return ZKFL_OK;
  const KeyGroups& g = k->grp;
  if (g.on && !(g.learned && 2 * (uint64_t)g.last_miss > g.non_rep)) return ZKFL_OK;
  if (J.w_ready) HIP_TRY(hipEventSynchronize(J.w_ready), "wait for the witness group");
  return key_learn_groups(ctx, k, J.w);
}

template <class GetJob>
int run_jobs(zkfl_ctx* ctx, size_t n, GetJob job) {
  HIP_TRY(hipSetDevice(ctx->device), "hipSetDevice");
  struct PerKey {
    zkfl_key* key;
    size_t issued = 0;
  };
  std::vector<PerKey> cursor;
  auto issue = [&](PerKey& pk, size_t i, const Job& J, const uint32_t* rsl) -> int {
    ProofSlot* s = nullptr;
    int rc = get_slot(J.key, pk.issued++, &s);
    if (rc) return rc;
    if (s->busy) {
      rc = wait_slot(s, n > 1);
      if (rc) return rc;
    }
    s->job = i;
    s->out_proof = J.part_out ? nullptr : J.proof_out;
    s->out_part = J.part_out;
    if (J.w_ready) {
      hipError_t e = hipStreamWaitEvent(s->st_main, J.w_ready, 0);
      if (e != hipSuccess) return hip_fail(e, "wait for the witness group");
    }
    rc = enqueue_proof(ctx, J.key, s, J.w, rsl, J.part_out ? ProofMode::SplitPart : ProofMode::Proof, n == 1);
    if (rc) return rc;
    s->busy = true;
    return ZKFL_OK;
  };
  int rc = ZKFL_OK;
  for (size_t i = 0; i < n && rc == ZKFL_OK; i++) {
    Job J;
    rc = job(i, J);
    if (rc) break;
    if (J.key->nshards != 1 && !J.part_out) {
      rc = fail(ZKFL_E_ARG, "this key is shard " + std::to_string(J.key->shard) + " of " +
                                std::to_string(J.key->nshards) +
                                " of a split proof: prove parts (zkfl_groth16_prove_part_batch) and assemble them");
      break;
    }
    uint32_t rsl[16];
    rc = get_rs(J.rs, rsl);
    if (rc) break;
    size_t c = 0;
    while (c < cursor.size() && cursor[c].key != J.key) c++;
    if (c == cursor.size()) {
      cursor.emplace_back();
      cursor.back().key = J.key;
      rc = learn_for_batch(ctx, J, n);
      if (rc) break;
    }
    rc = issue(cursor[c], i, J, rsl);
  }
  for (auto& pk : cursor) {
    for (ProofSlot* s : pk.key->slots)
      if (s->busy) {
        int r2 = wait_slot(s, n > 1);
        if (rc == ZKFL_OK) rc = r2;
      }
  }
  return rc;
}

}

extern "C" {

int zkfl_groth16_prove_resident(zkfl_ctx* ctx, zkfl_key* key, const zkfl_witness* w, const uint8_t* rs,
                                uint8_t proof_out[256]) {
  return zkfl_groth16_prove_batch(ctx, key, 1, &w, rs, proof_out);
}

int zkfl_key_set_slots(zkfl_key* key, int slots) {
  if (!key || slots < 1 || slots > 32) return fail(ZKFL_E_ARG, "slots must be in 1..32");
  (void)hipSetDevice(key->ctx->device);
  for (ProofSlot* s : key->slots) {
    if (s->busy) return fail(ZKFL_E_ARG, "slots busy");
  }
  while ((int)key->slots.size() > slots) {
    slot_release(key->slots.back());
    key->slots.pop_back();
  }
  if (slots > 1)
    for (ProofSlot* s : key->slots) slot_drop_lowlat(s);
  key->max_slots = slots;
  return ZKFL_OK;
}

int zkfl_groth16_prove_batch(zkfl_ctx* ctx, zkfl_key* key, size_t n, const zkfl_witness* const* w,
                             const uint8_t* rs, uint8_t* proofs_out) {
  if (!ctx || !key || (!w && n) || (!proofs_out && n)) return fail(ZKFL_E_ARG, "null argument");
  for (size_t i = 0; i < n; i++) {
    if (!w[i] || w[i]->key != key) return fail(ZKFL_E_MISMATCH, "witness uploaded for another key");
  }
  return run_jobs(ctx, n, [&](size_t i, Job& J) {
    J.key = key;
    J.w = w[i]->d;
    J.rs = rs ? rs + 64 * i : nullptr;
    J.proof_out = proofs_out + 256 * i;
    return ZKFL_OK;
  });
}

int zkfl_groth16_prove_part_batch(zkfl_ctx* ctx, zkfl_key* key, size_t n, const zkfl_witness* const* w,
                                  const uint8_t* rs, uint8_t* parts_out) {
  if (!ctx || !key || (n && (!w || !rs || !parts_out))) return fail(ZKFL_E_ARG, "prove_part: null argument");
  for (size_t i = 0; i < n; i++) {
    if (!w[i] || w[i]->key != key) return fail(ZKFL_E_MISMATCH, "witness uploaded for another key");
  }
  return run_jobs(ctx, n, [&](size_t i, Job& J) {
    J.key = key;
    J.w = w[i]->d;
    J.rs = rs + 64 * i;
    J.part_out = parts_out + PART_WORDS * 4 * i;
    return ZKFL_OK;
  });
}

int zkfl_groth16_assemble(zkfl_ctx* ctx, size_t n, size_t n_parts, const uint8_t* parts, const uint8_t* rs,
                          uint8_t* proofs_out) {
  if (!ctx || (n && (!parts || !rs || !proofs_out)) || n_parts < 1 || n_parts > 1024)
    return fail(ZKFL_E_ARG, "assemble: bad arguments");
  if (n == 0) return ZKFL_OK;
  for (size_t i = 0; i < n * n_parts * (PART_WORDS / 8); i++)
    if (!fq_lt_q(reinterpret_cast<const uint32_t*>(parts + 32 * i)))
      return fail(ZKFL_E_ARG, "assemble: part coordinate " + std::to_string(i) + " is not < q");
  std::vector<uint8_t> ks(n * 4 * sizeof(GlvScalar));
  for (size_t i = 0; i < n; i++) {
    uint32_t rsl[16];
    int rc = get_rs(rs + 64 * i, rsl);
// ... 235 lines not shown
    }
    cv.notify_all();
    for (auto& t : th) t.join();
  }
  void work() {
    for (;;) {
      const size_t i = next.fetch_add(1);
      if (i >= n) return;
      {
        std::unique_lock<std::mutex> g(mu);
        cv.wait(g, [&] { return stop || i < consumed + AHEAD; });
        if (stop) return;
      }
      std::vector<uint32_t> v;
      std::string e;
      int r = texts[i] ? wprog_inputs_json(prog, texts[i], v, e) : ZKFL_E_ARG;
      if (!texts[i]) e = "null input json";
      if (r == ZKFL_OK && v.size() != n_in * 8) {
        r = ZKFL_E_ARG;
        e = "input json does not fill the program's inputs";
      }
      v.resize(n_in * 8 + 8);
      {
        std::lock_guard<std::mutex> g(mu);
        vec[i] = std::move(v);
        err[i] = std::move(e);
        rc[i] = r;
        done[i] = 1;
      }
      cv.notify_all();
    }
  }
  int get(size_t i, const uint8_t** out) {
    std::unique_lock<std::mutex> g(mu);
    if (i > 0) std::vector<uint32_t>().swap(vec[i - 1]);
    consumed = i;
    cv.notify_all();
    cv.wait(g, [&] { return done[i] != 0; });
    if (rc[i]) return fail(rc[i], "input " + std::to_string(i) + ": " + err[i]);
    *out = reinterpret_cast<const uint8_t*>(vec[i].data());
    return ZKFL_OK;
  }
};
}

int zkfl_groth16_full_prove_json_batch(zkfl_ctx* ctx, zkfl_key* key, const zkfl_wprog* prog, size_t n,
                                       const char* const* input_jsons, const uint8_t* rs, uint8_t* proofs_out,
                                       uint8_t* pubs_out) {
  if (!ctx || (n && (!input_jsons || !proofs_out))) return fail(ZKFL_E_ARG, "full_prove_json_batch: null argument");
  size_t n_in = 0;
  int rc = full_prove_check(ctx, key, prog, 0, nullptr, &n_in);
  if (rc || n == 0) return rc;
  JsonParsePool pool(prog->p, input_jsons, n, n_in);
  return full_prove_piped(
      ctx, n, [&](size_t) { return key; }, [&](size_t) { return (const WProg*)prog->p; },
      [&](size_t i, const uint8_t** in) { return pool.get(i, in); }, rs, proofs_out,
      [&](size_t i) { return pubs_out ? pubs_out + (size_t)key->nPub * 32 * i : nullptr; });
}

int zkfl_groth16_full_prove_multi(zkfl_ctx* ctx, size_t n, zkfl_key* const* keys, const zkfl_wprog* const* progs,
                                  const uint8_t* const* inputs, const uint8_t* rs, uint8_t* proofs_out,
                                  uint8_t* const* pubs_out) {
  if (!ctx || (n && (!keys || !progs || !inputs || !proofs_out))) return fail(ZKFL_E_ARG, "full_prove_multi: null argument");
  std::vector<size_t> n_in(n);
  for (size_t i = 0; i < n; i++) {
    int rc = full_prove_check(ctx, keys[i], progs[i], 1, inputs[i], &n_in[i]);
    if (rc) return fail(rc, "job " + std::to_string(i) + ": " + zkfl_last_error());
  }
  std::vector<std::pair<const zkfl_key*, const zkfl_wprog*>> kp;
  for (size_t i = 0; i < n; i++) {
    size_t c = 0;
    while (c < kp.size() && kp[c].first != keys[i]) c++;
    if (c == kp.size()) kp.push_back({keys[i], progs[i]});
    else if (kp[c].second != progs[i])
      return fail(ZKFL_E_ARG, "full_prove_multi: job " + std::to_string(i) +
                                  " uses its key with another witness program than an earlier job");
  }
  return full_prove_piped(
      ctx, n, [&](size_t i) { return keys[i]; }, [&](size_t i) { return (const WProg*)progs[i]->p; },
      [&](size_t i, const uint8_t** in) {
        *in = inputs[i];
        return ZKFL_OK;
      },
      rs, proofs_out, [&](size_t i) { return pubs_out ? pubs_out[i] : nullptr; });
}

int zkfl_groth16_prove(zkfl_ctx* ctx, zkfl_key* key, const uint8_t* wtns, size_t wtns_len, const uint8_t* rs,
                       uint8_t proof_out[256], uint8_t* pub_out, size_t* npub) {
  zkfl_witness* w = nullptr;
  int rc = zkfl_witness_upload(ctx, key, wtns, wtns_len, &w);
  if (rc) return rc;
  rc = zkfl_groth16_prove_resident(ctx, key, w, rs, proof_out);
  if (rc == ZKFL_OK) {
    if (pub_out) memcpy(pub_out, w->pub.data(), w->pub.size());
    if (npub) *npub = key->nPub;
  }
  zkfl_witness_free(w);
  return rc;
}

int zkfl_debug_prove_parts(zkfl_ctx* ctx, zkfl_key* key, const uint8_t* wtns, size_t wtns_len, uint8_t* h_out,
                           uint8_t* msm_out) {
  zkfl_witness* w = nullptr;
  int rc = zkfl_witness_upload(ctx, key, wtns, wtns_len, &w);
  if (rc) return rc;
  ProofSlot* s = nullptr;
  rc = get_slot(key, 0, &s);
  uint32_t zeros[16] = {0};
  if (rc == ZKFL_OK && !key->dbg_zero) {
    const size_t bytes = std::max<size_t>(key->nVars, (size_t)key->n + 4) * 32;
    hipError_t e = hipMalloc(&key->dbg_zero, bytes);
    if (e == hipSuccess) e = hipMemsetAsync(key->dbg_zero, 0, bytes, s->st_main);
    if (e == hipSuccess) e = hipStreamSynchronize(s->st_main);
    if (e != hipSuccess) rc = hip_fail(e, "parity hook zeros");
  }
  if (rc == ZKFL_OK && s->busy) rc = wait_slot(s);
  if (rc == ZKFL_OK) {
    s->out_proof = nullptr;
    s->out_part = nullptr;
    rc = enqueue_proof(ctx, key, s, w->d, zeros, ProofMode::Parts, false);
  }
  if (rc == ZKFL_OK) rc = wait_slot(s);
  hipStream_t st = s ? s->st_main : ctx->st;
  uint32_t* d_o = nullptr;
  if (rc == ZKFL_OK && msm_out) {
    hipError_t e = hipMalloc(&d_o, 64 * 4 + 128);
    if (e == hipSuccess) {
      point_out(st, s->res, 4, d_o);
      point_out(st, s->resB2, 1, d_o + 64);
      e = hipGetLastError();
    }
    std::vector<uint8_t> tmp(64 * 4 + 128);
    if (e == hipSuccess) e = hipMemcpyAsync(tmp.data(), d_o, tmp.size(), hipMemcpyDeviceToHost, st);
    if (e == hipSuccess) e = hipStreamSynchronize(st);
    if (e != hipSuccess) rc = hip_fail(e, "debug parts");
    if (rc == ZKFL_OK) {
      memcpy(msm_out, tmp.data(), 64);
      memcpy(msm_out + 64, tmp.data() + 64, 64);
      memcpy(msm_out + 128, tmp.data() + 256, 128);
      memcpy(msm_out + 256, tmp.data() + 128, 64);
      memcpy(msm_out + 320, tmp.data() + 192, 64);
    }
  }
  if (rc == ZKFL_OK && h_out) {
    hipError_t e = hipMemcpyAsync(h_out, s->h, (size_t)key->n * 32, hipMemcpyDeviceToHost, st);
    if (e == hipSuccess) e = hipStreamSynchronize(st);
    if (e != hipSuccess) rc = hip_fail(e, "debug h");
  }
  if (d_o) (void)hipFree(d_o);
  zkfl_witness_free(w);
  return rc;
}

}
```

### verifiable-federated-training-with-zero-knowledge-proofs-zk-fl-_amd/csrc/zkfl.hip

```cpp
#include <hip/hip_runtime.h>
#include <stdint.h>
#include <string.h>
#include <sys/random.h>

#include <algorithm>
#include <cstdlib>
#include <string>
#include <type_traits>
#include <vector>

#include "assemble.h"
#include "devbufs.h"
#include "glv.h"
#include "host_parse.h"
#include "merkle.h"
#include "objects.h"
#include "poly.h"
#include "setup.h"
#include "verify.h"
#include "witness.h"

using namespace zkfl;

static thread_local std::string g_err;
// ... 43 lines not shown
  HIP_TRY(D.get(&d_s, n * 8), where);
  HIP_TRY(D.get(&d_r, 1), where);
  HIP_TRY(D.get(&d_o, 1), where);
  HIP_TRY(hipMemcpyAsync(d_b, bases, n * sizeof(Affine<F>), hipMemcpyHostToDevice, st), where);
  HIP_TRY(hipMemcpyAsync(d_s, scalars, n * 32, hipMemcpyHostToDevice, st), where);
  HIP_TRY(msm_bases_set(E.mb, d_b, nullptr, 0xFFFFFFFFu, st), where);
  HIP_TRY(msm_run(E.mb, E.ms, E.mt, d_s, nullptr, d_r, st, &ctx->prof,
                  std::is_same<F, FqOps>::value ? "msm_accumulate_g1" : "msm_accumulate_g2"),
          where);
  point_out(st, d_r, 1, reinterpret_cast<uint32_t*>(d_o));
  HIP_TRY(hipGetLastError(), where);
  HIP_TRY(hipMemcpyAsync(out, d_o, sizeof(Affine<F>), hipMemcpyDeviceToHost, st), where);
  HIP_TRY(hipStreamSynchronize(st), where);
  return ZKFL_OK;
}

int pos_ready(zkfl_ctx* ctx) {
  if (ctx->pos) return ZKFL_OK;
  std::string err;
  int rc = pos_tables_create(&ctx->pos, ctx->st, err);
  return rc ? fail(rc, err) : ZKFL_OK;
}

int check_fr_array(const uint8_t* v, size_t count, const char* what) {
  for (size_t i = 0; i < count; i++) {
    uint32_t w[8];
    memcpy(w, v + 32 * i, 32);
    if (!fr_lt_r(w)) return fail(ZKFL_E_ARG, std::string(what) + " " + std::to_string(i) + " is not < r");
  }
  return ZKFL_OK;
}

int tree_from_device_leaves(zkfl_ctx* ctx, DevBufs& B, const Fr* d_leaves, size_t n, uint32_t depth,
                            uint8_t* tree_out) {
  hipStream_t st = ctx->st;
  const size_t nodes = ((size_t)2 << depth) - 1;
  Fr *d_work, *d_tree;
  HIP_TRY(B.get(&d_work, merkle_work_size(n, depth)), "alloc");
  HIP_TRY(B.get(&d_tree, nodes), "alloc");
  int pi = ctx->prof.begin("merkle", st);
  HIP_TRY(merkle_build(ctx->pos, d_leaves, n, depth, d_tree, d_work, st), "merkle");
  ctx->prof.end(pi, st, (double)(merkle_work_size(n, depth) - n));
  HIP_TRY(hipMemcpyAsync(tree_out, d_tree, nodes * 32, hipMemcpyDeviceToHost, st), "download");
  HIP_TRY(hipStreamSynchronize(st), "sync");
  return ZKFL_OK;
}

int tree_args(zkfl_ctx* ctx, size_t n, uint32_t depth, const void* in, const void* out) {
  if (!ctx || !out || (n && !in)) return fail(ZKFL_E_ARG, "merkle: null argument");
  if (depth > ZKFL_MERKLE_MAX_DEPTH) return fail(ZKFL_E_ARG, "merkle: depth must be <= 30");
  if (n > ((size_t)1 << depth)) return fail(ZKFL_E_ARG, "merkle: more leaves than 2^depth");
  return ZKFL_OK;
}

}

void zkfl::ctx_retain(zkfl_ctx* ctx) { ctx->refs.fetch_add(1, std::memory_order_relaxed); }

void zkfl::ctx_release(zkfl_ctx* ctx) {
  if (ctx->refs.fetch_sub(1, std::memory_order_acq_rel) != 1) return;
  (void)hipSetDevice(ctx->device);
  (void)hipStreamSynchronize(ctx->st);
  ctx->prof.reset();
  vk_free(ctx->vk);
  pos_tables_free(ctx->pos);
  if (ctx->asm_buf) (void)hipFree(ctx->asm_buf);
  if (ctx->wt.rec) {
    (void)zkfl_debug_wtrace(ctx, 0, 0, nullptr, nullptr);
  }
  (void)hipStreamDestroy(ctx->st);
  delete ctx;
}

extern "C" {

int zkfl_version(void) { return 1; }

int zkfl_debug_glv_split(const uint8_t k[32], uint8_t out[40]) {
  if (!k || !out) return fail(ZKFL_E_ARG, "null argument");
  uint32_t kk[8];
  memcpy(kk, k, 32);
  if (!fr_lt_r(kk)) return fail(ZKFL_E_ARG, "k must be < r");
  GlvScalar a, b;
  glv_split(kk, a, b);
  memcpy(out, a.mag, 16);
  memcpy(out + 16, &a.neg, 4);
  memcpy(out + 20, b.mag, 16);
  memcpy(out + 36, &b.neg, 4);
  return ZKFL_OK;
}

int zkfl_debug_g1_glv_mul(zkfl_ctx* ctx, size_t n, const uint8_t* points, const uint8_t* scalars, uint8_t* out) {
  if (!ctx || (n && (!points || !scalars || !out))) return fail(ZKFL_E_ARG, "null argument");
  if (n == 0) return ZKFL_OK;
  if (n > (1u << 20)) return fail(ZKFL_E_ARG, "glv mul: n too large");
  std::vector<GlvScalar> ks(2 * n);
  for (size_t i = 0; i < n; i++) {
    uint32_t kk[8];
    memcpy(kk, scalars + 32 * i, 32);
    if (!fr_lt_r(kk)) return fail(ZKFL_E_ARG, "glv mul: scalar " + std::to_string(i) + " is not < r");
    glv_split(kk, ks[2 * i], ks[2 * i + 1]);
  }
  HIP_TRY(hipSetDevice(ctx->device), "hipSetDevice");
  hipStream_t st = ctx->st;
  DevBufs D;
  uint32_t *d_p, *d_o;
  GlvScalar* d_k;
  HIP_TRY(D.get(&d_p, n * 16), "glv mul");
  HIP_TRY(D.get(&d_k, ks.size()), "glv mul");
  HIP_TRY(D.get(&d_o, n * 16), "glv mul");
  HIP_TRY(hipMemcpyAsync(d_p, points, n * 64, hipMemcpyHostToDevice, st), "glv mul");
  HIP_TRY(hipMemcpyAsync(d_k, ks.data(), ks.size() * sizeof(GlvScalar), hipMemcpyHostToDevice, st), "glv mul");
  debug_glv_mul(st, (uint32_t)n, d_p, d_k, d_o);
  HIP_TRY(hipGetLastError(), "glv mul");
  HIP_TRY(hipMemcpyAsync(out, d_o, n * 64, hipMemcpyDeviceToHost, st), "glv mul");
  HIP_TRY(hipStreamSynchronize(st), "glv mul");
  return ZKFL_OK;
}

const char* zkfl_last_error(void) { return g_err.c_str(); }

int zkfl_device_count(int* count) {
  if (!count) return fail(ZKFL_E_ARG, "null");
  int c = 0;
  hipError_t e = hipGetDeviceCount(&c);
  if (e != hipSuccess) {
    *count = 0;
    return hip_fail(e, "hipGetDeviceCount");
  }
  *count = c;
  return ZKFL_OK;
}

int zkfl_ctx_create(int device, zkfl_ctx** out) {
  if (!out) return fail(ZKFL_E_ARG, "null out");
  int c = 0;
  if (hipGetDeviceCount(&c) != hipSuccess || c == 0) return fail(ZKFL_E_DEVICE, "no HIP device available");
  if (device < 0 || device >= c) return fail(ZKFL_E_ARG, "device index out of range");
  HIP_TRY(hipSetDevice(device), "hipSetDevice");
  zkfl_ctx* ctx = new zkfl_ctx();
  ctx->device = device;
  auto env = [](const char* name, int dflt) {
    const char* v = getenv(name);
    return v ? atoi(v) : dflt;
  };
  ctx->opts.graph = env("ZKFL_GRAPH", 1) != 0;
  ctx->opts.stagger = env("ZKFL_STAGGER", 1) != 0;
  ctx->opts.lowlat = env("ZKFL_LOWLAT", 1) != 0;
  ctx->opts.fast_wsum = env("ZKFL_FAST_WSUM", 1) != 0;
  ctx->opts.small_logn = env("ZKFL_SMALL_LOGN", 16);
  ctx->opts.ab_shared = env("ZKFL_AB_SHARED", 1) != 0;
  ctx->opts.groups = env("ZKFL_GROUPS", 1) != 0;
  ctx->opts.group_min_batch = std::max(1, env("ZKFL_GROUP_MIN_BATCH", 8));
  hipError_t e = hipStreamCreateWithFlags(&ctx->st, hipStreamNonBlocking);
  if (e != hipSuccess) {
    delete ctx;
    return hip_fail(e, "hipStreamCreate");
  }
  *out = ctx;
  return ZKFL_OK;
}

int zkfl_ctx_destroy(zkfl_ctx* ctx) {
  if (!ctx) return ZKFL_OK;
  (void)hipSetDevice(ctx->device);
  (void)hipStreamSynchronize(ctx->st);
  ctx_release(ctx);
  return ZKFL_OK;
}

int zkfl_ctx_set_profiling(zkfl_ctx* ctx, int enabled) {
  if (!ctx) return fail(ZKFL_E_ARG, "null ctx");
  ctx->prof.on = enabled != 0;
  ctx->prof.serialize = enabled == 2;
  return ZKFL_OK;
}

int zkfl_ctx_profile(zkfl_ctx* ctx, const char* name, double* total_ms, uint64_t* launches, double* units,
                     double* median_ms) {
  if (!ctx || !name || !total_ms || !launches) return fail(ZKFL_E_ARG, "null");
  (void)hipSetDevice(ctx->device);
  HIP_TRY(hipDeviceSynchronize(), "sync");
  ctx->prof.query(name, total_ms, launches, units, median_ms);
  return ZKFL_OK;
}

int zkfl_ctx_profile_reset(zkfl_ctx* ctx) {
  if (!ctx) return fail(ZKFL_E_ARG, "null ctx");
  (void)hipStreamSynchronize(ctx->st);
  ctx->prof.reset();
  return ZKFL_OK;
}

int zkfl_ctx_synchronize(zkfl_ctx* ctx) {
  if (!ctx) return fail(ZKFL_E_ARG, "null ctx");
  HIP_TRY(hipSetDevice(ctx->device), "hipSetDevice");
  HIP_TRY(hipDeviceSynchronize(), "sync");
  return ZKFL_OK;
}

int zkfl_witness_upload(zkfl_ctx* ctx, const zkfl_key* key, const uint8_t* wtns, size_t wtns_len,
                        zkfl_witness** out) {
  if (!ctx || !key || !wtns || !out) return fail(ZKFL_E_ARG, "null argument");
  WtnsView v;
  int rc = parse_wtns(wtns, wtns_len, v);
  if (rc) return rc;
  if (v.n != key->nVars) return fail(ZKFL_E_MISMATCH, "wtns: nWitness != zkey nVars");
  HIP_TRY(hipSetDevice(ctx->device), "hipSetDevice");
  zkfl_witness* w = new zkfl_witness();
  w->key = key;
  hipError_t e = hipMalloc(&w->d, (size_t)v.n * 32);
  if (e == hipSuccess) e = hipMemcpyAsync(w->d, v.data, (size_t)v.n * 32, hipMemcpyHostToDevice, ctx->st);
  if (e == hipSuccess) e = hipStreamSynchronize(ctx->st);
  if (e != hipSuccess) {
    zkfl_witness_free(w);
    return hip_fail(e, "witness upload");
  }
  w->pub.assign(v.data + 32, v.data + 32 + (size_t)key->nPub * 32);
  *out = w;
  return ZKFL_OK;
}

int zkfl_witness_free(zkfl_witness* w) {
  if (!w) return ZKFL_OK;
  if (w->d) (void)hipFree(w->d);
  delete w;
  return ZKFL_OK;
}

int zkfl_debug_wtrace(zkfl_ctx* ctx, int op, uint32_t cap, void* out, uint32_t* count) {
#if !ZK_WTRACE
  (void)ctx;
  (void)op;
  (void)cap;
  (void)out;
  (void)count;
  return fail(ZKFL_E_ARG, "wave trace: this library was built without -DZK_WTRACE=1");
#else
  if (!ctx || op < 0 || op > 2) return fail(ZKFL_E_ARG, "wave trace: bad arguments");
  HIP_TRY(hipSetDevice(ctx->device), "hipSetDevice");
  auto bind_all = [](const WtBuf& b) {
    hipError_t e = zk_wtrace_bind_poly(b);
    if (e == hipSuccess) e = zk_wtrace_bind_asm(b);
    if (e == hipSuccess) e = zk_wtrace_bind_g1(b);
    if (e == hipSuccess) e = zk_wtrace_bind_g2(b);
    if (e == hipSuccess) e = zk_wtrace_bind_sort(b);
    if (e == hipSuccess) e = zk_wtrace_bind_ntt(b);
    if (e == hipSuccess) e = zk_wtrace_bind_wit(b);
    if (e == hipSuccess) e = zk_wtrace_bind_joint(b);
    return e;
  };
  HIP_TRY(hipDeviceSynchronize(), "wave trace: sync");
  if (op == 2) {
    if (!ctx->wt.rec) return fail(ZKFL_E_ARG, "wave trace: not started");
    uint32_t n = 0;
    HIP_TRY(hipMemcpy(&n, ctx->wt.cnt, 4, hipMemcpyDeviceToHost), "wave trace: count");
    HIP_TRY(bind_all(WtBuf()), "wave trace: unbind");
    const uint32_t m = std::min(n, std::min(cap, ctx->wt.cap));
    if (out && m) HIP_TRY(hipMemcpy(out, ctx->wt.rec, (size_t)m * sizeof(WtRec), hipMemcpyDeviceToHost), "wave trace: read");
    if (count) *count = n;
    return ZKFL_OK;
  }
  HIP_TRY(bind_all(WtBuf()), "wave trace: unbind");
  if (ctx->wt.rec) (void)hipFree(ctx->wt.rec);
  if (ctx->wt.cnt) (void)hipFree(ctx->wt.cnt);
  ctx->wt = WtBuf();
  if (op == 0) return ZKFL_OK;
  if (cap == 0) return fail(ZKFL_E_ARG, "wave trace: cap must be > 0");
  HIP_TRY(hipMalloc(&ctx->wt.rec, (size_t)cap * sizeof(WtRec)), "wave trace: alloc");
  HIP_TRY(hipMalloc(&ctx->wt.cnt, 4), "wave trace: alloc");
  HIP_TRY(hipMemset(ctx->wt.cnt, 0, 4), "wave trace: reset");
  ctx->wt.cap = cap;
  HIP_TRY(bind_all(ctx->wt), "wave trace: bind");
  HIP_TRY(hipDeviceSynchronize(), "wave trace: sync");
  return ZKFL_OK;
#endif
}

int zkfl_msm_g1(zkfl_ctx* ctx, const uint8_t* bases, const uint8_t* scalars, size_t n, uint8_t out[64]) {
  return run_msm_primitive<FqOps>(ctx, bases, scalars, n, out);
}

int zkfl_msm_g2(zkfl_ctx* ctx, const uint8_t* bases, const uint8_t* scalars, size_t n, uint8_t out[128]) {
  return run_msm_primitive<Fq2Ops>(ctx, bases, scalars, n, out);
}

int zkfl_debug_ntt_coset(zkfl_ctx* ctx, uint8_t* data, uint32_t logn, uint32_t nvec, size_t vstride, int col_max) {
  if (!ctx || !data || logn < 1 || logn > 27 || nvec < 1 || nvec > 3 || col_max > NTT_COL_TILE_LOG)
    return fail(ZKFL_E_ARG, "ntt: bad args");
  const size_t n = (size_t)1 << logn;
  if (vstride < n || vstride > ((size_t)1 << 32)) return fail(ZKFL_E_ARG, "ntt: bad stride");
  hipStream_t st = ctx->st;
  struct Plan {
    NttPlan pl;
    ~Plan() { ntt_plan_free(pl); }
  } P;
  DevBufs D;
  Fr* d;
  const size_t count = (size_t)(nvec - 1) * vstride + n;
  HIP_TRY(ntt_plan_alloc(P.pl, (int)logn, st), "ntt");
  if (col_max >= 0) P.pl.col_max = col_max;
  HIP_TRY(D.get(&d, count), "ntt");
  HIP_TRY(hipMemcpyAsync(d, data, count * 32, hipMemcpyHostToDevice, st), "ntt");
  for (uint32_t v = 0; v < nvec; v++) fr_std_to_mont(st, d + v * vstride, n);
  HIP_TRY(ntt_coset_shift(P.pl, d, (int)nvec, vstride, st), "ntt");
  for (uint32_t v = 0; v < nvec; v++) fr_mont_to_std(st, d + v * vstride, n);
// ... 575 lines not shown
```

### verifiable-federated-training-with-zero-knowledge-proofs-zk-fl-_amd/zkfl/native.py

```python

from __future__ import annotations

import ctypes as C
import os

_PKG_DIR = os.path.dirname(os.path.dirname(os.path.abspath(__file__)))
LIB_PATH = os.path.abspath(os.environ["ZKFL_LIB"]) if os.environ.get("ZKFL_LIB") else os.path.join(_PKG_DIR, "libzkfl.so")

ZKFL_OK = 0
PART_BYTES = 768
PART_LAYOUT = {"A": (0, 128), "B1": (128, 256), "B2": (256, 512), "C": (512, 640), "H": (640, 768)}
ERRORS = {
    -1: "ZKFL_E_ARG", -2: "ZKFL_E_FORMAT", -3: "ZKFL_E_PRIME", -4: "ZKFL_E_MISMATCH",
    -5: "ZKFL_E_DEVICE", -6: "ZKFL_E_OOM", -7: "ZKFL_E_CONSTRAINT", -8: "ZKFL_E_KEY",
}

_P = C.c_void_p
_U8P = C.POINTER(C.c_uint8)


class R1csHeader(C.Structure):
    _fields_ = [("n_wires", C.c_uint32), ("n_pub_out", C.c_uint32), ("n_pub_in", C.c_uint32),
                ("n_prv_in", C.c_uint32), ("n_constraints", C.c_uint32), ("n_labels", C.c_uint64),
                ("n_terms", C.c_uint64)]

    def as_dict(self) -> dict:
        return {k: int(getattr(self, k)) for k, _ in self._fields_}


class R1csReport(C.Structure):
    _fields_ = [("n_failed", C.c_uint32), ("first", C.c_uint32), ("a", C.c_uint8 * 32), ("b", C.c_uint8 * 32),
                ("c", C.c_uint8 * 32)]


class PtauView(C.Structure):
    _fields_ = [("power", C.c_uint32),
                ("L", C.c_char_p), ("L2", C.c_char_p), ("La", C.c_char_p), ("Lb", C.c_char_p), ("H0", C.c_char_p),
                ("L_len", C.c_size_t), ("L2_len", C.c_size_t), ("La_len", C.c_size_t), ("Lb_len", C.c_size_t),
                ("H0_len", C.c_size_t),
                ("alpha1", C.c_char_p), ("beta1", C.c_char_p), ("beta2", C.c_char_p)]


KEY_CHECKS = ("header", "points", "coefficients", "A", "B1", "B2", "IC", "C", "H")
KEY_STATES = ("pass", "fail", "not run")


class ZkeyReport(C.Structure):
    _fields_ = [("status", C.c_uint32 * len(KEY_CHECKS)),
                ("point_section", C.c_uint32), ("point_index", C.c_uint32), ("point_count", C.c_uint32),
                ("coef_matrix", C.c_uint32), ("coef_row", C.c_uint32), ("coef_count", C.c_uint32)]


GROUP_QUERIES = ("A", "B1", "B2", "CH")


class GroupsInfo(C.Structure):
    _fields_ = [("grouped", C.c_uint32), ("learned", C.c_uint32), ("groups", C.c_uint32), ("non_rep", C.c_uint32),
                ("bases", C.c_uint32 * 4), ("bases_rep", C.c_uint32 * 4), ("builds", C.c_uint32),
                ("last_miss", C.c_uint32), ("build_ms", C.c_double)]


SIGNATURES = {
    "zkfl_version": (C.c_int, []),
    "zkfl_build_id": (C.c_char_p, []),
    "zkfl_last_error": (C.c_char_p, []),
    "zkfl_device_count": (C.c_int, [C.POINTER(C.c_int)]),
    "zkfl_ctx_create": (C.c_int, [C.c_int, C.POINTER(_P)]),
    "zkfl_ctx_destroy": (C.c_int, [_P]),
    "zkfl_ctx_set_profiling": (C.c_int, [_P, C.c_int]),
    "zkfl_ctx_profile": (C.c_int, [_P, C.c_char_p, C.POINTER(C.c_double), C.POINTER(C.c_uint64),
                                   C.POINTER(C.c_double), C.POINTER(C.c_double)]),
    "zkfl_ctx_profile_reset": (C.c_int, [_P]),
    "zkfl_ctx_synchronize": (C.c_int, [_P]),
    "zkfl_zkey_load": (C.c_int, [_P, C.c_char_p, C.c_size_t, C.POINTER(_P)]),
    "zkfl_zkey_load_shard": (C.c_int, [_P, C.c_char_p, C.c_size_t, C.c_uint32, C.c_uint32, C.POINTER(_P)]),
    "zkfl_zkey_file_open": (C.c_int, [C.c_char_p, C.POINTER(_P)]),
    "zkfl_zkey_load_file": (C.c_int, [_P, _P, C.POINTER(_P)]),
    "zkfl_zkey_file_close": (C.c_int, [_P]),
    "zkfl_key_shard": (C.c_int, [_P, C.POINTER(C.c_uint32), C.POINTER(C.c_uint32)]),
    "zkfl_groth16_prove_part_batch": (C.c_int, [_P, _P, C.c_size_t, C.POINTER(_P), C.c_char_p, _U8P]),
    "zkfl_groth16_assemble": (C.c_int, [_P, C.c_size_t, C.c_size_t, C.c_char_p, C.c_char_p, _U8P]),
    "zkfl_key_free": (C.c_int, [_P]),
    "zkfl_key_info": (C.c_int, [_P, C.POINTER(C.c_uint32), C.POINTER(C.c_uint32), C.POINTER(C.c_uint32)]),
    "zkfl_key_ab_shared": (C.c_int, [_P, C.POINTER(C.c_uint32), C.POINTER(C.c_uint32), C.POINTER(C.c_uint32)]),
    "zkfl_debug_ab_partition": (C.c_int, [C.c_char_p, C.c_char_p, C.c_size_t, C.c_uint32, C.c_uint32,
                                          C.POINTER(C.c_uint32), C.POINTER(C.c_uint32), _U8P]),
    "zkfl_key_set_groups": (C.c_int, [_P, C.POINTER(C.c_uint32), C.c_size_t]),
    "zkfl_key_learn_groups": (C.c_int, [_P, _P, _P]),
    "zkfl_key_groups": (C.c_int, [_P, C.POINTER(GroupsInfo)]),
    "zkfl_debug_groups": (C.c_int, [C.c_char_p, C.c_char_p, C.c_size_t, C.POINTER(C.c_uint32), C.POINTER(C.c_uint32),
                                    C.c_size_t, C.c_uint32, C.POINTER(C.c_uint32), C.POINTER(C.c_uint32),
                                    C.POINTER(C.c_uint32)]),
    "zkfl_key_set_slots": (C.c_int, [_P, C.c_int]),
    "zkfl_groth16_prove": (C.c_int, [_P, _P, C.c_char_p, C.c_size_t, C.c_char_p, _U8P, _U8P,
                                     C.POINTER(C.c_size_t)]),
    "zkfl_witness_upload": (C.c_int, [_P, _P, C.c_char_p, C.c_size_t, C.POINTER(_P)]),
    "zkfl_witness_free": (C.c_int, [_P]),
    "zkfl_groth16_prove_resident": (C.c_int, [_P, _P, _P, C.c_char_p, _U8P]),
    "zkfl_groth16_prove_batch": (C.c_int, [_P, _P, C.c_size_t, C.POINTER(_P), C.c_char_p, _U8P]),
    "zkfl_debug_prove_parts": (C.c_int, [_P, _P, C.c_char_p, C.c_size_t, _U8P, _U8P]),
    "zkfl_debug_glv_split": (C.c_int, [C.c_char_p, _U8P]),
    "zkfl_debug_g1_glv_mul": (C.c_int, [_P, C.c_size_t, C.c_char_p, C.c_char_p, _U8P]),
    "zkfl_debug_wtrace": (C.c_int, [_P, C.c_int, C.c_uint32, _P, C.POINTER(C.c_uint32)]),
    "zkfl_msm_g1": (C.c_int, [_P, C.c_char_p, C.c_char_p, C.c_size_t, _U8P]),
    "zkfl_msm_g2": (C.c_int, [_P, C.c_char_p, C.c_char_p, C.c_size_t, _U8P]),
    "zkfl_ntt_coset": (C.c_int, [_P, _U8P, C.c_uint32]),
    "zkfl_debug_ntt_coset": (C.c_int, [_P, _U8P, C.c_uint32, C.c_uint32, C.c_size_t, C.c_int]),
    "zkfl_setup_g1_gen_mul": (C.c_int, [_P, C.c_char_p, C.c_size_t, _U8P]),
    "zkfl_setup_g2_gen_mul": (C.c_int, [_P, C.c_char_p, C.c_size_t, _U8P]),
    "zkfl_setup_g1_scale": (C.c_int, [_P, C.c_char_p, C.c_char_p, C.c_size_t, _U8P]),
    "zkfl_setup_g2_scale": (C.c_int, [_P, C.c_char_p, C.c_char_p, C.c_size_t, _U8P]),
    "zkfl_setup_g1_lagrange": (C.c_int, [_P, C.c_char_p, C.c_uint32, _U8P]),
    "zkfl_setup_g2_lagrange": (C.c_int, [_P, C.c_char_p, C.c_uint32, _U8P]),
    "zkfl_setup_g1_lincomb": (C.c_int, [_P, C.c_char_p, C.c_size_t, C.c_size_t, C.POINTER(C.c_uint64),
                                        C.POINTER(C.c_uint32), C.c_char_p, _U8P]),
    "zkfl_setup_g2_lincomb": (C.c_int, [_P, C.c_char_p, C.c_size_t, C.c_size_t, C.POINTER(C.c_uint64),
                                        C.POINTER(C.c_uint32), C.c_char_p, _U8P]),
    "zkfl_groth16_verify": (C.c_int, [_P, C.c_char_p, C.c_size_t, C.c_char_p, C.c_size_t, C.c_char_p]),
    "zkfl_groth16_verify_batch": (C.c_int, [_P, C.c_char_p, C.c_size_t, C.c_size_t, C.c_char_p, C.c_size_t,
                                            C.c_char_p, C.POINTER(C.c_int32)]),
    "zkfl_pairing": (C.c_int, [_P, C.c_size_t, C.c_char_p, C.c_char_p, _U8P]),
    "zkfl_debug_miller_loop": (C.c_int, [_P, C.c_size_t, C.c_char_p, C.c_char_p, _U8P]),
    "zkfl_vkey_load": (C.c_int, [_P, C.c_char_p, C.c_size_t, C.POINTER(_P)]),
    "zkfl_vkey_info": (C.c_int, [_P, C.POINTER(C.c_uint32)]),
    "zkfl_vkey_free": (C.c_int, [_P]),
    "zkfl_groth16_verify_multi": (C.c_int, [_P, C.c_size_t, C.POINTER(_P), C.POINTER(C.c_char_p),
                                            C.POINTER(C.c_size_t), C.c_char_p, C.POINTER(C.c_int32), C.c_int]),
    "zkfl_groth16_verify_round": (C.c_int, [_P, C.c_size_t, C.POINTER(_P), C.POINTER(C.c_char_p),
                                            C.POINTER(C.c_size_t), C.c_char_p, C.c_char_p, C.POINTER(C.c_int32),
                                            C.POINTER(C.c_uint32)]),
    "zkfl_debug_verify_round": (C.c_int, [_P, C.c_size_t, C.POINTER(_P), C.POINTER(C.c_char_p),
                                          C.POINTER(C.c_size_t), C.c_char_p, C.c_char_p, C.c_size_t, _U8P,
                                          C.POINTER(C.c_int32)]),
    "zkfl_debug_wave_pairing": (C.c_int,[_P, C.c_size_t, C.c_char_p, C.c_char_p, C.c_int, _U8P]),
    "zkfl_wprog_load": (C.c_int, [_P, C.c_char_p, C.c_size_t, C.POINTER(_P)]),
    "zkfl_wprog_free": (C.c_int, [_P]),
    "zkfl_wprog_info": (C.c_int, [_P, C.POINTER(C.c_uint32), C.POINTER(C.c_uint32), C.POINTER(C.c_uint32)]),
    "zkfl_wtns_size": (C.c_size_t, [_P]),
    "zkfl_witness_compute": (C.c_int, [_P, _P, C.c_size_t, C.c_char_p, _U8P]),
    "zkfl_witness_compute_resident": (C.c_int, [_P, _P, _P, C.c_size_t, C.c_char_p, C.POINTER(_P)]),
    "zkfl_wprog_parse_inputs": (C.c_int, [C.c_char_p, C.c_size_t, C.c_char_p, _U8P, C.c_size_t,
                                          C.POINTER(C.c_size_t)]),
    "zkfl_witness_compute_json": (C.c_int, [_P, _P, C.c_char_p, _U8P]),
    "zkfl_groth16_full_prove_batch": (C.c_int, [_P, _P, _P, C.c_size_t, C.c_char_p, C.c_char_p, _U8P, _U8P]),
    "zkfl_poseidon_params": (C.c_int, [C.c_uint32, _U8P, _U8P, C.POINTER(C.c_uint32)]),
    "zkfl_poseidon_batch": (C.c_int, [_P, C.c_uint32, C.c_size_t, C.c_char_p, _U8P]),
    "zkfl_vector_hash_batch": (C.c_int, [_P, C.c_uint32, C.c_size_t, C.c_char_p, _U8P]),
    "zkfl_merkle_build": (C.c_int, [_P, C.c_char_p, C.c_size_t, C.c_uint32, _U8P]),
    "zkfl_dataset_commit": (C.c_int, [_P, C.c_char_p, C.c_size_t, C.c_uint32, C.c_uint32, _U8P]),
    "zkfl_groth16_full_prove_json": (C.c_int, [_P, _P, _P, C.c_char_p, C.c_char_p, _U8P, _U8P]),
    "zkfl_groth16_prove_multi": (C.c_int, [_P, C.c_size_t, C.POINTER(_P), C.POINTER(_P), C.c_char_p, _U8P]),
    "zkfl_groth16_full_prove_json_batch": (C.c_int, [_P, _P, _P, C.c_size_t, C.POINTER(C.c_char_p), C.c_char_p, _U8P,
                                                     _U8P]),
    "zkfl_groth16_full_prove_multi": (C.c_int, [_P, C.c_size_t, C.POINTER(_P), C.POINTER(_P), C.POINTER(C.c_char_p),
                                                C.c_char_p, _U8P, C.POINTER(_U8P)]),
    "zkfl_r1cs_parse": (C.c_int, [C.c_char_p, C.c_size_t, C.POINTER(R1csHeader)]),
    "zkfl_r1cs_load": (C.c_int, [_P, C.c_char_p, C.c_size_t, C.POINTER(_P)]),
    "zkfl_r1cs_info": (C.c_int, [_P, C.POINTER(R1csHeader)]),
    "zkfl_r1cs_free": (C.c_int, [_P]),
    "zkfl_r1cs_check": (C.c_int, [_P, _P, C.c_size_t, C.POINTER(C.c_char_p), C.POINTER(C.c_size_t),
                                  C.POINTER(R1csReport)]),
    "zkfl_r1cs_check_resident": (C.c_int, [_P, _P, C.c_size_t, C.POINTER(_P), C.POINTER(R1csReport)]),
    "zkfl_zkey_check": (C.c_int, [_P, _P, C.c_char_p, C.c_size_t, C.POINTER(PtauView), C.c_char_p, C.c_char_p,
                                  C.POINTER(ZkeyReport)]),
}


class ZkflError(RuntimeError):
    def __init__(self, code, msg):
        super().__init__(f"{ERRORS.get(code, code)}: {msg}")
        self.code = code


_lib = None


def lib():
    global _lib
    if _lib is None:
        if not os.path.exists(LIB_PATH):
            raise ZkflError(-5, f"{LIB_PATH} not built (run make in the package dir / __graft_entry__.build())")
        L = C.CDLL(LIB_PATH)
        ab = bool(os.environ.get("ZKFL_LIB"))
        for name, (res, args) in SIGNATURES.items():
            if ab and not hasattr(L, name):
                continue
            fn = getattr(L, name)
            fn.restype = res
            fn.argtypes = args
        _lib = L
    return _lib


def check(rc):
    if rc != ZKFL_OK:
        raise ZkflError(rc, lib().zkfl_last_error().decode(errors="replace"))


def _frs(values) -> bytes:
    return b"".join(int(v).to_bytes(32, "little") for v in values)


def _ints(b: bytes) -> list:
    return [int.from_bytes(b[i:i + 32], "little") for i in range(0, len(b), 32)]


def _levels(flat, depth):
    out, pos = [], 0
    for lvl in range(depth + 1):
        w = 1 << (depth - lvl)
        out.append(flat[pos:pos + w])
        pos += w
    return out


def poseidon_params(t: int):
    c = _buf(32 * (8 + 70) * t)
    xy = _buf(64 * t)
    rp = C.c_uint32()
    check(lib().zkfl_poseidon_params(t, c, xy, C.byref(rp)))
    consts = _ints(bytes(c))[:(8 + rp.value) * t]
    pts = _ints(bytes(xy))
    return consts, pts[:t], pts[t:], rp.value


def build_id() -> str:
    return lib().zkfl_build_id().decode()


def source_id(pkg_dir: str = _PKG_DIR) -> str:
    import glob
    import hashlib
    names = sorted(os.path.relpath(p, pkg_dir) for ext in ("h", "hip", "cc")
                   for p in glob.glob(os.path.join(pkg_dir, "csrc", "*." + ext)))
    h = hashlib.sha256()
    for n in names + [os.path.join("..", "include", "zkfl.h")]:
        with open(os.path.join(pkg_dir, n), "rb") as f:
            h.update(f.read())
    return h.hexdigest()[:16]


def device_count() -> int:
    n = C.c_int(0)
    if lib().zkfl_device_count(C.byref(n)) != ZKFL_OK:
        return 0
# ... 231 lines not shown
        n, keys, pubs, npubs, proofs, z = self._round_args(jobs, z)
        out = _buf(384)
        scr = (C.c_int32 * max(1, n))()
        check(lib().zkfl_debug_verify_round(self.h, n, keys, pubs, npubs, proofs, z, chunk, out, scr))
        return bytes(out)[:384], [bool(scr[i]) for i in range(n)]

    def wave_pairing(self, g1: bytes, g2: bytes, final_exp: bool = True) -> bytes:
        n = len(g1) // 64
        assert len(g1) == 64 * n and len(g2) == 128 * n
        out = _buf(384 * n if n else 1)
        check(lib().zkfl_debug_wave_pairing(self.h, n, g1, g2, 1 if final_exp else 0, out))
        return bytes(out)[:384 * n]

    def poseidon_batch(self, rows) -> list:
        if not rows:
            return []
        arity = len(rows[0])
        assert all(len(r) == arity for r in rows)
        out = _buf(32 * len(rows))
        check(lib().zkfl_poseidon_batch(self.h, arity, len(rows), _frs(v for r in rows for v in r), out))
        return _ints(bytes(out))

    def vector_hash_batch(self, vectors) -> list:
        if not vectors:
            return []
        ln = len(vectors[0])
        assert all(len(v) == ln for v in vectors)
        out = _buf(32 * len(vectors))
        check(lib().zkfl_vector_hash_batch(self.h, ln, len(vectors), _frs(x for v in vectors for x in v), out))
        return _ints(bytes(out))

    def merkle_build(self, leaves, depth: int) -> list:
        out = _buf(32 * ((2 << depth) - 1))
        check(lib().zkfl_merkle_build(self.h, _frs(leaves), len(leaves), depth, out))
        return _levels(_ints(bytes(out)), depth)

    def dataset_commit(self, samples, depth: int) -> list:
        ln = len(samples[0]) if samples else 1
        assert all(len(v) == ln for v in samples)
        flat = self.dataset_commit_raw(_frs(x for v in samples for x in v), len(samples), ln, depth)
        return _levels(_ints(flat), depth)

    def dataset_commit_raw(self, values: bytes, n: int, ln: int, depth: int) -> bytes:
        assert len(values) == 32 * n * ln
        out = _buf(32 * ((2 << depth) - 1))
        check(lib().zkfl_dataset_commit(self.h, values, n, ln, depth, out))
        return bytes(out)

    def prove_multi(self, jobs, rs: bytes | None = None) -> list:
        n = len(jobs)
        keys = (_P * max(1, n))(*[k.h for k, _ in jobs])
        ws = (_P * max(1, n))(*[w.h for _, w in jobs])
        out = _buf(256 * max(1, n))
        check(lib().zkfl_groth16_prove_multi(self.h, n, keys, ws, rs, out))
        return _proofs(out, n)

    def full_prove_multi(self, jobs, rs: bytes | None = None) -> list:
        n = len(jobs)
        for k, wp, inp in jobs:
            if len(inp) != 32 * wp.n_inputs:
                raise ZkflError(-1, f"expected {wp.n_inputs} input values (32 B each)")
        keys = (_P * max(1, n))(*[k.h for k, _, _ in jobs])
        progs = (_P * max(1, n))(*[wp.h for _, wp, _ in jobs])
        ins = (C.c_char_p * max(1, n))(*[inp for _, _, inp in jobs])
        pub_bufs = [_buf(32 * max(1, k.n_public)) for k, _, _ in jobs]
        pubs = (_U8P * max(1, n))(*[C.cast(b, _U8P) for b in pub_bufs])
        out = _buf(256 * max(1, n))
        check(lib().zkfl_groth16_full_prove_multi(self.h, n, keys, progs, ins, rs, out, pubs))
        return [(p, _ints(bytes(pub_bufs[i]))[:jobs[i][0].n_public]) for i, p in enumerate(_proofs(out, n))]

    def assemble(self, parts: bytes, n_parts: int, rs: bytes) -> list:
        n = len(rs) // 64
        if len(rs) != 64 * n or len(parts) != PART_BYTES * n * n_parts:
            raise ZkflError(-1, "assemble: parts / rs sizes disagree")
        out = _buf(256 * max(1, n))
        check(lib().zkfl_groth16_assemble(self.h, n, n_parts, parts, rs, out))
        return _proofs(out, n)

    def pairing(self, g1: bytes, g2: bytes, final_exp: bool = True) -> bytes:
        n = len(g1) // 64
        assert len(g1) == 64 * n and len(g2) == 128 * n
        out = _buf(384 * n if n else 1)
        fn = lib().zkfl_pairing if final_exp else lib().zkfl_debug_miller_loop
        check(fn(self.h, n, g1, g2, out))
        return bytes(out)[:384 * n]


VERIFY_SCHEDULES = {"auto": 0, "lanes": 1, "waves": 2}
ROUND_REPORT_FIELDS = ("keys", "screened", "combined", "passed", "fallback")


class VerifyingKey(_Handle):
    _free = "zkfl_vkey_free"

    def __init__(self, ctx: Context, vk_bytes: bytes):
        h = _P()
        check(lib().zkfl_vkey_load(ctx.h, vk_bytes, len(vk_bytes), C.byref(h)))
        self.h = h
        self.ctx = ctx
        ctx._own(self)
        npub = C.c_uint32()
        check(lib().zkfl_vkey_info(h, C.byref(npub)))
        self.n_public = npub.value


class ProvingKey(_Handle):
    _free = "zkfl_key_free"

    def __init__(self, ctx: Context, zkey, shard: int = 0, n_shards: int = 1):
        h = _P()
        if isinstance(zkey, (str, os.PathLike)):
            if (shard, n_shards) != (0, 1):
                with open(zkey, "rb") as f:
                    zkey = f.read()
            else:
                fh = _P()
                check(lib().zkfl_zkey_file_open(os.fsencode(zkey), C.byref(fh)))
                try:
                    check(lib().zkfl_zkey_load_file(ctx.h, fh, C.byref(h)))
                finally:
                    lib().zkfl_zkey_file_close(fh)
        if h:
            pass
        elif n_shards == 1 and shard == 0:
            check(lib().zkfl_zkey_load(ctx.h, zkey, len(zkey), C.byref(h)))
        else:
            check(lib().zkfl_zkey_load_shard(ctx.h, zkey, len(zkey), shard, n_shards, C.byref(h)))
        self.h = h
        self.shard, self.n_shards = shard, n_shards
        self.ctx = ctx
        ctx._own(self)
        nv, npub, dom = C.c_uint32(), C.c_uint32(), C.c_uint32()
        check(lib().zkfl_key_info(h, C.byref(nv), C.byref(npub), C.byref(dom)))
        self.n_vars, self.n_public, self.domain_size = nv.value, npub.value, dom.value

    def ab_shared(self) -> dict:
        d, sh, nb = C.c_uint32(), C.c_uint32(), C.c_uint32()
        check(lib().zkfl_key_ab_shared(self.h, C.byref(d), C.byref(sh), C.byref(nb)))
        return {"form": "D" if d.value else "A", "shared_wires": sh.value, "a_bases": nb.value}

    def set_groups(self, rep):
        if rep is None:
            check(lib().zkfl_key_set_groups(self.h, None, 0))
            return
        arr = (C.c_uint32 * max(1, len(rep)))(*rep)
        check(lib().zkfl_key_set_groups(self.h, arr, len(rep)))

    def learn_groups(self, w: "ResidentWitness"):
        check(lib().zkfl_key_learn_groups(self.ctx.h, self.h, w.h))

    def groups(self) -> dict:
        g = GroupsInfo()
        check(lib().zkfl_key_groups(self.h, C.byref(g)))
        return {"grouped": bool(g.grouped), "learned": bool(g.learned), "groups": g.groups, "non_rep": g.non_rep,
                "bases": dict(zip(GROUP_QUERIES, g.bases)), "bases_rep": dict(zip(GROUP_QUERIES, g.bases_rep)),
                "builds": g.builds, "last_miss": g.last_miss, "build_ms": g.build_ms}

    def set_slots(self, slots: int):
        check(lib().zkfl_key_set_slots(self.h, slots))
        self.slots = slots

    def prove(self, wtns: bytes, rs: bytes | None = None):
        proof = _buf(256)
        pub = _buf(32 * max(1, self.n_public))
        npub = C.c_size_t()
        check(lib().zkfl_groth16_prove(self.ctx.h, self.h, wtns, len(wtns), rs, proof, pub, C.byref(npub)))
        pb = bytes(pub)
        return bytes(proof), [int.from_bytes(pb[32 * i:32 * i + 32], "little") for i in range(npub.value)]

    def upload(self, wtns: bytes) -> "ResidentWitness":
        return ResidentWitness(self, wtns)

    def prove_resident(self, w: "ResidentWitness", rs: bytes | None = None) -> bytes:
        proof = _buf(256)
        check(lib().zkfl_groth16_prove_resident(self.ctx.h, self.h, w.h, rs, proof))
        return bytes(proof)

    def prove_batch(self, ws, rs: bytes | None = None) -> list:
        n = len(ws)
        arr = (_P * n)(*[w.h for w in ws])
        out = _buf(256 * n)
        check(lib().zkfl_groth16_prove_batch(self.ctx.h, self.h, n, arr, rs, out))
        return _proofs(out, n)

    def prove_part_batch(self, ws, rs: bytes) -> list:
        n = len(ws)
        if rs is None or len(rs) != 64 * n:
            raise ZkflError(-1, "prove_part_batch: rs must be n x 64 bytes")
        arr = (_P * max(1, n))(*[w.h for w in ws])
        out = _buf(PART_BYTES * max(1, n))
        check(lib().zkfl_groth16_prove_part_batch(self.ctx.h, self.h, n, arr, rs, out))
        ob = bytes(out)
        return [ob[PART_BYTES * i:PART_BYTES * (i + 1)] for i in range(n)]

    def full_prove_batch(self, prog: "WitnessProgram", inputs, rs: bytes | None = None):
        n = len(inputs)
        buf = prog._inputs(inputs)
        out = _buf(256 * max(1, n))
        pubs = _buf(32 * max(1, self.n_public) * max(1, n))
        check(lib().zkfl_groth16_full_prove_batch(self.ctx.h, self.h, prog.h, n, buf, rs, out, pubs))
        return _proofs_publics(out, pubs, n, self.n_public)

    def full_prove_json_batch(self, prog: "WitnessProgram", texts, rs: bytes | None = None):
        n = len(texts)
        arr = (C.c_char_p * max(1, n))(*[t.encode() if isinstance(t, str) else t for t in texts])
        out = _buf(256 * max(1, n))
        pubs = _buf(32 * max(1, self.n_public) * max(1, n))
        check(lib().zkfl_groth16_full_prove_json_batch(self.ctx.h, self.h, prog.h, n, arr, rs, out, pubs))
        return _proofs_publics(out, pubs, n, self.n_public)

    def full_prove_json(self, prog: "WitnessProgram", input_json: str, rs: bytes | None = None):
        out = _buf(256)
        pub = _buf(32 * max(1, self.n_public))
        check(lib().zkfl_groth16_full_prove_json(self.ctx.h, self.h, prog.h, input_json.encode(), rs, out, pub))
        return bytes(out), _ints(bytes(pub))[:self.n_public]

    def debug_parts(self, wtns: bytes):
        h = _buf(32 * self.domain_size)
        m = _buf(384)
        check(lib().zkfl_debug_prove_parts(self.ctx.h, self.h, wtns, len(wtns), h, m))
        hb, mb = bytes(h), bytes(m)
        hs = [int.from_bytes(hb[32 * i:32 * i + 32], "little") for i in range(self.domain_size)]
        parts = dict(A=mb[0:64], B1=mb[64:128], B2=mb[128:256], C=mb[256:320], H=mb[320:384])
        return hs, parts


class ResidentWitness(_Handle):
    _free = "zkfl_witness_free"

    def __init__(self, key: ProvingKey, wtns: bytes | None = None, handle=None):
        if handle is not None:
            self.h = handle
            key.ctx._own(self)
            return
        h = _P()
        check(lib().zkfl_witness_upload(key.ctx.h, key.h, wtns, len(wtns), C.byref(h)))
        self.h = h
        key.ctx._own(self)


def parse_inputs(image: bytes, input_json: str, cap: int | None = None) -> bytes:
    if cap is None:
        cap = max(1, int.from_bytes(image[16:20], "little") + int.from_bytes(image[20:24], "little"))
    out = _buf(32 * cap)
    n = C.c_size_t()
    check(lib().zkfl_wprog_parse_inputs(image, len(image), input_json.encode(), out, cap, C.byref(n)))
    return bytes(out)[:32 * n.value]


class WitnessProgram(_Handle):
    _free = "zkfl_wprog_free"

    def __init__(self, ctx: Context, image: bytes):
        h = _P()
        check(lib().zkfl_wprog_load(ctx.h, image, len(image), C.byref(h)))
        self.h, self.ctx = h, ctx
        ctx._own(self)
        nw, ni, npub = C.c_uint32(), C.c_uint32(), C.c_uint32()
        check(lib().zkfl_wprog_info(h, C.byref(nw), C.byref(ni), C.byref(npub)))
        self.n_wires, self.n_inputs, self.n_public = nw.value, ni.value, npub.value
        self.wtns_size = lib().zkfl_wtns_size(h)

    def _inputs(self, inputs) -> bytes:
        buf = b"".join(inputs)
        if len(buf) != 32 * self.n_inputs * len(inputs):
            raise ZkflError(-1, f"expected {self.n_inputs} input values (32 B each) per witness")
        return buf

    def compute(self, inputs) -> list:
        n = len(inputs)
        out = _buf(self.wtns_size * max(1, n))
        check(lib().zkfl_witness_compute(self.ctx.h, self.h, n, self._inputs(inputs), out))
        ob = bytes(out)
        return [ob[i * self.wtns_size:(i + 1) * self.wtns_size] for i in range(n)]

    def compute_json(self, input_json: str) -> bytes:
        out = _buf(self.wtns_size)
        check(lib().zkfl_witness_compute_json(self.ctx.h, self.h, input_json.encode(), out))
        return bytes(out)

    def compute_resident(self, key: ProvingKey, inputs) -> list:
        n = len(inputs)
        arr = (_P * max(1, n))()
        check(lib().zkfl_witness_compute_resident(self.ctx.h, self.h, key.h, n, self._inputs(inputs), arr))
        return [ResidentWitness(key, handle=_P(arr[i])) for i in range(n)]


NO_CONSTRAINT = 0xFFFFFFFF


class Report:

    def __init__(self, r: R1csReport):
        self.n_failed, self.first = int(r.n_failed), int(r.first)
        self.a, self.b, self.c = (int.from_bytes(bytes(x), "little") for x in (r.a, r.b, r.c))

    @property
    def ok(self) -> bool:
        return self.n_failed == 0

    def __repr__(self):
        if self.ok:
            return "Report(ok)"
        return f"Report(n_failed={self.n_failed}, first={self.first}, a={self.a}, b={self.b}, c={self.c})"


def r1cs_header(r1cs: bytes) -> dict:
    h = R1csHeader()
    check(lib().zkfl_r1cs_parse(r1cs, len(r1cs), C.byref(h)))
# ... 72 lines not shown
```

Baseline: 814.7 proofs/s.

## Deduplicate R1CS A/B rows into classes and recompute only rows dirtied by group misses

```diff
diff --git a/include/zkfl.h b/include/zkfl.h
--- a/include/zkfl.h
+++ b/include/zkfl.h
@@ -58,12 +58,30 @@
   uint32_t last_miss;
   double build_ms;
 } zkfl_groups_info;
+typedef struct zkfl_group_rows_info {
+  uint32_t rows_grouped;
+  uint32_t row_classes;
+  uint32_t terms;
+  uint32_t terms_rep;
+  uint32_t wire_list;
+  uint32_t wires_over_cap;
+  uint32_t last_dirty;
+  uint32_t last_plain;
+  double rows_build_ms;
+} zkfl_group_rows_info;
 int zkfl_key_set_groups(zkfl_key* key, const uint32_t* rep, size_t n_vars);
 int zkfl_key_learn_groups(zkfl_ctx* ctx, zkfl_key* key, const zkfl_witness* w);
 int zkfl_key_groups(const zkfl_key* key, zkfl_groups_info* out);
+int zkfl_key_group_rows(const zkfl_key* key, zkfl_group_rows_info* out);
 int zkfl_debug_groups(const uint8_t* values, const uint8_t* sig, size_t n, uint32_t* rep_out, const uint32_t* sidx,
                       size_t n_bases, uint32_t u_base, uint32_t* sidx_out, uint32_t* start_out,
                       uint32_t* members_out);
+int zkfl_debug_group_rows(const uint32_t* rows, uint32_t domain, const uint32_t* cols, uint32_t cshift,
+                          const uint32_t* coefs, const uint32_t* rep, uint32_t n_vars, uint32_t hash_bits,
+                          uint32_t wire_cap, uint32_t* cls_out, uint32_t* crp_out, uint32_t* cterms_out,
+                          uint32_t* ccoefs_out, uint32_t* wstart_out, uint32_t* wlist_out, uint32_t* info_out);
+int zkfl_debug_abc(zkfl_ctx* ctx, zkfl_key* key, const zkfl_witness* w, int grouped, uint8_t* abc_out,
+                   uint32_t* counts_out);
 int zkfl_key_set_slots(zkfl_key* key, int slots);
 
 int zkfl_groth16_prove(zkfl_ctx* ctx, zkfl_key* key, const uint8_t* wtns, size_t wtns_len,
diff --git a/verifiable-federated-training-with-zero-knowledge-proofs-zk-fl-_amd/csrc/groups.h b/verifiable-federated-training-with-zero-knowledge-proofs-zk-fl-_amd/csrc/groups.h
--- a/verifiable-federated-training-with-zero-knowledge-proofs-zk-fl-_amd/csrc/groups.h
+++ b/verifiable-federated-training-with-zero-knowledge-proofs-zk-fl-_amd/csrc/groups.h
@@ -72,6 +72,133 @@
     if (to[j] != NONE) q.members[cur[to[j]]++] = (uint32_t)j;
 }
 
+
+constexpr uint32_t GROUP_ROWS_WIRE_CAP = 256;
+constexpr uint32_t GROUP_ROWS_DIRTY_DIV = 8;
+inline uint32_t group_rows_dirty_cap(uint32_t domain) { return std::max<uint32_t>(64u, domain / GROUP_ROWS_DIRTY_DIV); }
+constexpr uint32_t GROUP_ROWS_MISS_DIV = 64;
+inline uint32_t group_rows_miss_cap(uint32_t domain) { return std::max<uint32_t>(64u, domain / GROUP_ROWS_MISS_DIV); }
+constexpr uint32_t GROUP_ROWS_OVER = 0x80000000u;
+
+struct GroupRows {
+  std::vector<uint32_t> cls;
+  std::vector<uint32_t> crp;
+  std::vector<uint32_t> cterms;
+  std::vector<uint32_t> ccoefs;
+  std::vector<uint32_t> wstart;
+  std::vector<uint32_t> wlist;
+  uint32_t classes = 0;
+  uint32_t over_cap = 0;
+  bool keep = false;
+};
+
+inline void group_rows_build(const uint32_t* rows, uint32_t domain, const uint32_t* cols, uint32_t cshift,
+                             const uint32_t* coefs, const uint32_t* rep, uint32_t n_vars, uint32_t hash_bits,
+                             uint32_t wire_cap, GroupRows& g) {
+  const uint32_t nrows = 2 * domain, K = rows[nrows];
+  const uint32_t cmask = cshift ? (1u << cshift) - 1u : 0xFFFFFFFFu;
+  std::vector<uint64_t> key(K);
+  std::vector<uint32_t> uniq;
+  if (cshift) {
+    for (uint32_t p = 0; p < K; p++) key[p] = (cols[p] & ~cmask) | rep[cols[p] & cmask];
+  } else {
+    struct H32 {
+      const uint32_t* c;
+      size_t operator()(uint32_t p) const {
+        uint64_t h = 1469598103934665603ull;
+        for (int k = 0; k < 8; k++) h = (h ^ c[8 * (size_t)p + k]) * 1099511628211ull;
+        return (size_t)h;
+      }
+    };
+    struct E32 {
+      const uint32_t* c;
+      bool operator()(uint32_t a, uint32_t b) const { return memcmp(c + 8 * (size_t)a, c + 8 * (size_t)b, 32) == 0; }
+    };
+    std::unordered_map<uint32_t, uint32_t, H32, E32> ids(16, H32{coefs}, E32{coefs});
+    for (uint32_t p = 0; p < K; p++) {
+      const auto it = ids.emplace(p, (uint32_t)uniq.size());
+      if (it.second) uniq.push_back(p);
+      key[p] = (uint64_t)it.first->second << 32 | rep[cols[p]];
+    }
+  }
+  std::vector<uint64_t> hash(nrows);
+  const uint64_t hmask = hash_bits >= 64 ? ~0ull : (1ull << hash_bits) - 1ull;
+  for (uint32_t r = 0; r < nrows; r++) {
+    std::sort(key.begin() + rows[r], key.begin() + rows[r + 1]);
+    uint64_t h = 0x9E3779B97F4A7C15ull + (rows[r + 1] - rows[r]);
+    for (uint32_t p = rows[r]; p < rows[r + 1]; p++) {
+      h = (h ^ key[p]) * 0xFF51AFD7ED558CCDull;
+      h ^= h >> 29;
+    }
+    hash[r] = h & hmask;
+  }
+  uint32_t tbits = 4;
+  while ((1ull << tbits) < 2ull * nrows) tbits++;
+  std::vector<uint32_t> table((size_t)1 << tbits, 0xFFFFFFFFu), first;
+  const size_t tmask = ((size_t)1 << tbits) - 1;
+  g.cls.assign(nrows, 0);
+  g.crp.assign(1, 0);
+  g.cterms.clear();
+  g.ccoefs.clear();
+  for (uint32_t r = 0; r < nrows; r++) {
+    const uint32_t s = rows[r], len = rows[r + 1] - s;
+    size_t slot = (size_t)((hash[r] * 0x9E3779B97F4A7C15ull) >> (64 - tbits)) & tmask;
+    uint32_t c;
+    for (;; slot = (slot + 1) & tmask) {
+      c = table[slot];
+      if (c == 0xFFFFFFFFu) break;
+      const uint32_t f = first[c];
+      if (hash[f] == hash[r] && rows[f + 1] - rows[f] == len &&
+          std::equal(key.begin() + s, key.begin() + s + len, key.begin() + rows[f]))
+        break;
+    }
+    if (c == 0xFFFFFFFFu) {
+      c = table[slot] = (uint32_t)first.size();
+      first.push_back(r);
+      for (uint32_t p = s; p < s + len; p++) {
+        g.cterms.push_back((uint32_t)key[p]);
+        if (!cshift) {
+          const uint32_t* v = coefs + 8 * (size_t)uniq[key[p] >> 32];
+          g.ccoefs.insert(g.ccoefs.end(), v, v + 8);
+        }
+      }
+      g.crp.push_back((uint32_t)g.cterms.size());
+    }
+    g.cls[r] = c;
+  }
+  g.classes = (uint32_t)first.size();
+  g.keep = 2 * (uint64_t)g.cterms.size() <= K;
+  constexpr uint32_t NONE = 0xFFFFFFFFu;
+  std::vector<uint32_t> last(n_vars, NONE), cnt(n_vars, 0);
+  auto walk = [&](auto&& hit) {
+    std::fill(last.begin(), last.end(), NONE);
+    for (uint32_t j = 0; j < domain; j++)
+      for (int ab = 0; ab < 2; ab++)
+        for (uint32_t p = rows[ab * domain + j]; p < rows[ab * domain + j + 1]; p++) {
+          const uint32_t i = cols[p] & cmask;
+          if (rep[i] == i || last[i] == j) continue;
+          last[i] = j;
+          hit(i, j);
+        }
+  };
+  walk([&](uint32_t i, uint32_t) { cnt[i]++; });
+  g.wstart.assign((size_t)n_vars + 1, 0);
+  g.over_cap = 0;
+  for (uint32_t i = 0; i < n_vars; i++) {
+    const bool over = cnt[i] > wire_cap;
+    g.over_cap += over;
+    if (over) cnt[i] = 0;
+    g.wstart[i + 1] = g.wstart[i] + cnt[i];
+    cnt[i] = over ? NONE : g.wstart[i];
+  }
+  g.wlist.assign(g.wstart[n_vars], 0);
+  walk([&](uint32_t i, uint32_t j) {
+    if (cnt[i] != NONE) g.wlist[cnt[i]++] = j;
+  });
+  for (uint32_t i = 0; i < n_vars; i++)
+    if (cnt[i] == NONE) g.wstart[i] |= GROUP_ROWS_OVER;
+}
+
 }
 
 #ifdef __HIPCC__
@@ -84,8 +211,21 @@
 template <class F>
 void group_sums(hipStream_t st, const Affine<F>* bases_w, int W, size_t n, const uint32_t* start,
                 const uint32_t* members, Affine<F>* out);
+struct GroupMark {
+  const uint32_t* wstart;
+  const uint32_t* wlist;
+  uint32_t* state;
+  uint32_t* missing;
+  uint32_t miss_cap;
+  uint32_t* dirty;
+  uint32_t cap;
+};
+constexpr uint32_t GROUP_ROWS_STATE_BITS = 3;
+inline size_t group_rows_state_words(size_t n) { return GROUP_ROWS_STATE_BITS + (n + 31) / 32; }
+
 void group_delta(hipStream_t st, const Fr* w, const uint32_t* rep, uint32_t n, Fr* u, uint32_t* cnt,
-                 uint32_t* miss_out);
+                 uint32_t* miss_out, const GroupMark& mark);
+void group_mark_rows(hipStream_t st, const GroupMark& mark);
 
 }
 #endif
diff --git a/verifiable-federated-training-with-zero-knowledge-proofs-zk-fl-_amd/csrc/groups.hip b/verifiable-federated-training-with-zero-knowledge-proofs-zk-fl-_amd/csrc/groups.hip
--- a/verifiable-federated-training-with-zero-knowledge-proofs-zk-fl-_amd/csrc/groups.hip
+++ b/verifiable-federated-training-with-zero-knowledge-proofs-zk-fl-_amd/csrc/groups.hip
@@ -49,7 +49,7 @@
 
 __global__ void __launch_bounds__(DELTA_T) k_group_delta(const Fr* __restrict__ w, const uint32_t* __restrict__ rep,
                                                          uint32_t n, Fr* __restrict__ u, uint32_t* __restrict__ cnt,
-                                                         uint32_t* __restrict__ miss_out) {
+                                                         uint32_t* __restrict__ miss_out, const GroupMark M) {
   ZK_LIGHT();
   const uint32_t i = blockIdx.x * DELTA_T + threadIdx.x;
   int nz = 0;
@@ -63,14 +63,54 @@
     }
     u[i] = v;
   }
+  if (M.wstart) {
+    const unsigned long long m = __ballot(nz);
+    if (m) {
+      const uint32_t lane = threadIdx.x & (warpSize - 1);
+      const int first = __ffsll((long long)m) - 1;
+      uint32_t base = 0;
+      if ((int)lane == first) base = atomicAdd(&M.state[2], (uint32_t)__popcll(m));
+      base = __shfl(base, first);
+      const uint32_t at = base + (uint32_t)__popcll(m & ((1ull << lane) - 1ull));
+      if (nz && at < M.miss_cap) M.missing[at] = i;
+    }
+  }
   const int blk = __syncthreads_count(nz);
   if (threadIdx.x == 0) {
     if (blk) atomicAdd(&cnt[0], (uint32_t)blk);
     __threadfence();
     if (atomicAdd(&cnt[1], 1u) == gridDim.x - 1) {
       __threadfence();
-      *miss_out = atomicExch(&cnt[0], 0u);
+      miss_out[0] = atomicExch(&cnt[0], 0u);
       cnt[1] = 0;
+    }
+  }
+}
+
+constexpr int MARK_T = 256, MARK_BLOCKS_MAX = 256;
+
+__global__ void __launch_bounds__(MARK_T) k_group_mark(const GroupMark M) {
+  ZK_LIGHT();
+  const uint32_t n = M.state[2];
+  if (n == 0) return;
+  if (n > M.miss_cap) {
+    if (blockIdx.x == 0 && threadIdx.x == 0) atomicExch(&M.state[1], 1u);
+    return;
+  }
+  const uint32_t lane = threadIdx.x & (warpSize - 1), per = MARK_T / warpSize;
+  for (uint32_t k = blockIdx.x * per + threadIdx.x / warpSize; k < n; k += gridDim.x * per) {
+    if (__any((int)__atomic_load_n(&M.state[1], __ATOMIC_RELAXED))) return;
+    const uint32_t i = M.missing[k], s = M.wstart[i], e = M.wstart[i + 1] & ~GROUP_ROWS_OVER;
+    if (s & GROUP_ROWS_OVER) {
+      if (lane == 0) atomicExch(&M.state[1], 1u);
+      return;
+    }
+    for (uint32_t p = s + lane; p < e; p += warpSize) {
+      const uint32_t j = M.wlist[p], bit = 1u << (j & 31);
+      if (atomicOr(&M.state[GROUP_ROWS_STATE_BITS + (j >> 5)], bit) & bit) continue;
+      const uint32_t at = atomicAdd(&M.state[0], 1u);
+      if (at < M.cap) M.dirty[at] = j;
+      else atomicExch(&M.state[1], 1u);
     }
   }
 }
@@ -88,8 +128,13 @@
 template void group_sums<Fq2Ops>(hipStream_t, const G2Aff*, int, size_t, const uint32_t*, const uint32_t*, G2Aff*);
 
 void group_delta(hipStream_t st, const Fr* w, const uint32_t* rep, uint32_t n, Fr* u, uint32_t* cnt,
-                 uint32_t* miss_out) {
-  hipLaunchKernelGGL(k_group_delta, dim3(zk_grid(n, DELTA_T)), dim3(DELTA_T), 0, st, w, rep, n, u, cnt, miss_out);
+                 uint32_t* miss_out, const GroupMark& mark) {
+  hipLaunchKernelGGL(k_group_delta, dim3(zk_grid(n, DELTA_T)), dim3(DELTA_T), 0, st, w, rep, n, u, cnt, miss_out, mark);
+}
+
+void group_mark_rows(hipStream_t st, const GroupMark& mark) {
+  const unsigned blocks = std::min<unsigned>(zk_grid((size_t)mark.miss_cap * 64, MARK_T), MARK_BLOCKS_MAX);
+  hipLaunchKernelGGL(k_group_mark, dim3(blocks), dim3(MARK_T), 0, st, mark);
 }
 
 void key_groups_release(zkfl_key* k) {
@@ -97,7 +142,10 @@
   msm_bases_free(k->gB1);
   msm_bases_free(k->gB2);
   msm_bases_free(k->gCH);
-  if (k->grp.d_rep) (void)hipFree(k->grp.d_rep);
+  void* ptrs[] = {k->grp.d_rep,    k->grp.d_cls,    k->grp.d_crp,  k->grp.d_cterms,
+                  k->grp.d_ccoefs, k->grp.d_wstart, k->grp.d_wlist};
+  for (void* p : ptrs)
+    if (p) (void)hipFree(p);
   const uint32_t builds = k->grp.builds;
   k->grp = KeyGroups();
   k->grp.builds = builds;
@@ -123,6 +171,51 @@
   group_sums<F>(st, plain.bases_w, msm_w_of(plain.c), plain.n, d_start, d_members, d_img);
   ZK_CHECK(hipGetLastError());
   return msm_bases_set(out, d_img, q.sidx.data(), extra_start, st, false);
+}
+
+bool group_rows_wanted(const zkfl_key* k) {
+  return k->ctx->opts.group_rows && k->K != 0 && k->logn > k->ctx->opts.small_logn;
+}
+
+hipError_t build_rows(zkfl_key* k, const std::vector<uint32_t>& rep, hipStream_t st) {
+  KeyGroups& g = k->grp;
+  if (!group_rows_wanted(k)) return hipSuccess;
+  const auto t0 = std::chrono::steady_clock::now();
+  const uint32_t dom = k->n;
+  const size_t K = k->K;
+  std::vector<uint32_t> rows(2 * (size_t)dom + 1), cols(K), coefs;
+  ZK_CHECK(hipMemcpyAsync(rows.data(), k->rows, rows.size() * 4, hipMemcpyDeviceToHost, st));
+  ZK_CHECK(hipMemcpyAsync(cols.data(), k->cols, K * 4, hipMemcpyDeviceToHost, st));
+  if (!k->cshift) {
+    coefs.resize(K * 8);
+    ZK_CHECK(hipMemcpyAsync(coefs.data(), k->coefs, K * 32, hipMemcpyDeviceToHost, st));
+  }
+  ZK_CHECK(hipStreamSynchronize(st));
+  GroupRows R;
+  const uint32_t low = (uint32_t)k->ctx->opts.group_rows_cap;
+  group_rows_build(rows.data(), dom, cols.data(), k->cshift, coefs.data(), rep.data(), k->nVars, 64,
+                   low ? std::min(low, GROUP_ROWS_WIRE_CAP) : GROUP_ROWS_WIRE_CAP, R);
+  g.row_classes = R.classes;
+  g.terms_rep = (uint32_t)R.cterms.size();
+  g.wire_list = (uint32_t)R.wlist.size();
+  g.over_cap = R.over_cap;
+  if (R.keep && !R.cterms.empty()) {
+    auto up = [&](auto*& dst, const std::vector<uint32_t>& v) -> hipError_t {
+      ZK_CHECK(hipMalloc(&dst, (v.size() ? v.size() : 1) * 4));
+      if (!v.empty()) ZK_CHECK(hipMemcpyAsync(dst, v.data(), v.size() * 4, hipMemcpyHostToDevice, st));
+      return hipSuccess;
+    };
+    ZK_CHECK(up(g.d_cls, R.cls));
+    ZK_CHECK(up(g.d_crp, R.crp));
+    ZK_CHECK(up(g.d_cterms, R.cterms));
+    if (!k->cshift) ZK_CHECK(up(g.d_ccoefs, R.ccoefs));
+    ZK_CHECK(up(g.d_wstart, R.wstart));
+    ZK_CHECK(up(g.d_wlist, R.wlist));
+    ZK_CHECK(hipStreamSynchronize(st));
+    g.rows_on = true;
+  }
+  g.rows_ms = std::chrono::duration<double, std::milli>(std::chrono::steady_clock::now() - t0).count();
+  return hipSuccess;
 }
 
 int key_build_groups(zkfl_key* k, std::vector<uint32_t>& rep, bool learned, double host_ms) {
@@ -153,6 +246,7 @@
     if (e == hipSuccess) e = build_query(k->bCH, k->gCH, q[3], X, D, st);
     const hipError_t es = hipStreamSynchronize(st);
     if (e == hipSuccess) e = es;
+    if (e == hipSuccess) e = build_rows(k, rep, st);
   }
   if (e != hipSuccess) {
     key_groups_release(k);
@@ -179,6 +273,11 @@
           "%s and built in %.1f ms\n",
           nV, g.groups, g.non_rep, g.bases[0], g.bases_rep[0], g.bases[1], g.bases_rep[1], g.bases[3], g.bases_rep[3],
           learned ? "learned" : "set", g.build_ms);
+  if (group_rows_wanted(k))
+    fprintf(stderr,
+            "zkfl: key of %u wires: %u row classes, terms %zu -> %u, wire lists %u entries (%u wires over the cap); "
+            "%s ABC, built in %.1f ms of the above\n",
+            nV, g.row_classes, k->K, g.terms_rep, g.wire_list, g.over_cap, g.rows_on ? "grouped" : "plain", g.rows_ms);
   return ZKFL_OK;
 }
 
@@ -243,6 +342,56 @@
   out->builds = g.builds;
   out->last_miss = g.last_miss;
   out->build_ms = g.build_ms;
+  return ZKFL_OK;
+}
+
+int zkfl_key_group_rows(const zkfl_key* key, zkfl_group_rows_info* out) {
+  if (!key || !out) return fail(ZKFL_E_ARG, "null argument");
+  const KeyGroups& g = key->grp;
+  *out = zkfl_group_rows_info();
+  out->rows_grouped = g.rows_on;
+  out->row_classes = g.row_classes;
+  out->terms = (uint32_t)key->K;
+  out->terms_rep = g.row_classes ? g.terms_rep : out->terms;
+  out->wire_list = g.wire_list;
+  out->wires_over_cap = g.over_cap;
+  out->last_dirty = g.last_dirty;
+  out->last_plain = g.last_plain;
+  out->rows_build_ms = g.rows_ms;
+  return ZKFL_OK;
+}
+
+int zkfl_debug_group_rows(const uint32_t* rows, uint32_t domain, const uint32_t* cols, uint32_t cshift,
+                          const uint32_t* coefs, const uint32_t* rep, uint32_t n_vars, uint32_t hash_bits,
+                          uint32_t wire_cap, uint32_t* cls_out, uint32_t* crp_out, uint32_t* cterms_out,
+                          uint32_t* ccoefs_out, uint32_t* wstart_out, uint32_t* wlist_out, uint32_t* info_out) {
+  if (!rows || !rep || !cls_out || !crp_out || !cterms_out || !wstart_out || !wlist_out || !info_out ||
+      cshift >= 32 || domain > 0x3FFFFFFFu)
+    return fail(ZKFL_E_ARG, "debug_group_rows: bad arguments");
+  const uint32_t K = rows[2 * (size_t)domain];
+  if (K && (!cols || (!cshift && !coefs))) return fail(ZKFL_E_ARG, "debug_group_rows: terms missing");
+  for (uint32_t r = 0; r < 2 * domain; r++)
+    if (rows[r] > rows[r + 1]) return fail(ZKFL_E_ARG, "debug_group_rows: row pointers must not descend");
+  if (!groups_valid(rep, n_vars)) return fail(ZKFL_E_ARG, "debug_group_rows: not a partition");
+  const uint32_t cmask = cshift ? (1u << cshift) - 1u : 0xFFFFFFFFu;
+  for (uint32_t p = 0; p < K; p++)
+    if ((cols[p] & cmask) >= n_vars) return fail(ZKFL_E_ARG, "debug_group_rows: column past the wires");
+  GroupRows R;
+  group_rows_build(rows, domain, cols, cshift, coefs, rep, n_vars, hash_bits, wire_cap ? wire_cap : GROUP_ROWS_WIRE_CAP,
+                   R);
+  auto put = [](uint32_t* dst, const std::vector<uint32_t>& v) {
+    if (dst && !v.empty()) memcpy(dst, v.data(), v.size() * 4);
+  };
+  put(cls_out, R.cls);
+  put(crp_out, R.crp);
+  put(cterms_out, R.cterms);
+  put(ccoefs_out, R.ccoefs);
+  put(wstart_out, R.wstart);
+  put(wlist_out, R.wlist);
+  info_out[0] = R.classes;
+  info_out[1] = (uint32_t)R.cterms.size();
+  info_out[2] = (uint32_t)R.wlist.size();
+  info_out[3] = R.keep;
   return ZKFL_OK;
 }
 
diff --git a/verifiable-federated-training-with-zero-knowledge-proofs-zk-fl-_amd/csrc/objects.h b/verifiable-federated-training-with-zero-knowledge-proofs-zk-fl-_amd/csrc/objects.h
--- a/verifiable-federated-training-with-zero-knowledge-proofs-zk-fl-_amd/csrc/objects.h
+++ b/verifiable-federated-training-with-zero-knowledge-proofs-zk-fl-_amd/csrc/objects.h
@@ -42,6 +42,8 @@
   bool ab_shared = true;
   bool groups = true;
   int group_min_batch = 8;
+  bool group_rows = true;
+  int group_rows_cap = 0;
 };
 
 struct zkfl_ctx {
@@ -73,8 +75,14 @@
   Fr* abc_tail = nullptr;
   Fr* h = nullptr;
   uint32_t* grp_cnt = nullptr;
+  uint32_t* gr_state = nullptr;
+  uint32_t* gr_dirty = nullptr;
+  uint32_t* gr_missing = nullptr;
+  Fr* cls_val = nullptr;
+  size_t cls_cap = 0;
   zkfl_key* key = nullptr;
   bool grouped_run = false;
+  bool rows_run = false;
   G1P* res = nullptr;
   G2P* resB2 = nullptr;
   Fr* d_rs = nullptr;
@@ -107,6 +115,15 @@
   uint32_t builds = 0;
   uint32_t last_miss = 0;
   uint32_t* d_rep = nullptr;
+  bool rows_on = false;
+  uint32_t row_classes = 0;
+  uint32_t terms_rep = 0;
+  uint32_t wire_list = 0;
+  uint32_t over_cap = 0;
+  double rows_ms = 0;
+  uint32_t last_dirty = 0, last_plain = 0;
+  uint32_t *d_cls = nullptr, *d_crp = nullptr, *d_cterms = nullptr, *d_wstart = nullptr, *d_wlist = nullptr;
+  Fr* d_ccoefs = nullptr;
 };
 
 struct zkfl_key {
diff --git a/verifiable-federated-training-with-zero-knowledge-proofs-zk-fl-_amd/csrc/poly.h b/verifiable-federated-training-with-zero-knowledge-proofs-zk-fl-_amd/csrc/poly.h
--- a/verifiable-federated-training-with-zero-knowledge-proofs-zk-fl-_amd/csrc/poly.h
+++ b/verifiable-federated-training-with-zero-knowledge-proofs-zk-fl-_amd/csrc/poly.h
@@ -24,6 +24,8 @@
   const uint64_t* w_src_host;
   uint4* w_dst;
   uint32_t w_nvec;
+  uint32_t* gr_state;
+  uint32_t gr_words;
 };
 
 constexpr int RS_WORDS = (64 + 4 * (int)sizeof(GlvScalar)) / 4;
@@ -49,6 +51,21 @@
 void abc_chunks(hipStream_t st, const uint32_t* rp, uint32_t nrows, const AbcTerms& T, const Fr* w, uint32_t K,
                 Fr* head, Fr* tail, Fr* abc);
 void abc_rows(hipStream_t st, const uint32_t* rp, size_t n, uint32_t K, const Fr* head, const Fr* tail, Fr* abc);
+
+struct AbcGrouped {
+  const uint32_t* crp;
+  uint32_t classes;
+  AbcTerms terms;
+  uint32_t Kd;
+  const uint32_t* cls;
+  Fr* cls_val;
+  const uint32_t* state;
+  const uint32_t* dirty;
+  uint32_t cap;
+  uint32_t* report;
+};
+void abc_grouped(hipStream_t st, const AbcGrouped& G, const uint32_t* rp, size_t n, const AbcTerms& T, const Fr* w,
+                 uint32_t K, Fr* head, Fr* tail, Fr* abc);
 void join_h(hipStream_t st, const Fr* abc, size_t n, Fr* h);
 void proof_start(hipStream_t st, const uint32_t* rs_host, uint32_t* d_rs, Fr* extra, int plain, uint32_t* res3,
                  const ProofStart& ps);
diff --git a/verifiable-federated-training-with-zero-knowledge-proofs-zk-fl-_amd/csrc/poly.hip b/verifiable-federated-training-with-zero-knowledge-proofs-zk-fl-_amd/csrc/poly.hip
--- a/verifiable-federated-training-with-zero-knowledge-proofs-zk-fl-_amd/csrc/poly.hip
+++ b/verifiable-federated-training-with-zero-knowledge-proofs-zk-fl-_amd/csrc/poly.hip
@@ -1,4 +1,6 @@
 #include "poly.h"
+
+#include <algorithm>
 
 #include "common.h"
 #include "msm_api.h"
@@ -9,11 +11,8 @@
 namespace {
 
 template <bool PACKED>
-__global__ void __launch_bounds__(64) k_abc_chunks(const uint32_t* __restrict__ rp, uint32_t nrows, AbcTerms T,
-                                                   const Fr* __restrict__ w, uint32_t K, Fr* __restrict__ head,
-                                                   Fr* __restrict__ tail, Fr* __restrict__ abc) {
-  ZK_WT(WT_ABC);
-  ZK_LIGHT();
+ZK_DEV void abc_chunk(const uint32_t* __restrict__ rp, uint32_t nrows, const AbcTerms& T, const Fr* __restrict__ w,
+                      uint32_t K, Fr* __restrict__ head, Fr* __restrict__ tail, Fr* __restrict__ abc) {
   const uint32_t c = blockIdx.x * blockDim.x + threadIdx.x;
   const uint32_t p0 = c * ABC_L;
   if (p0 >= K) return;
@@ -66,11 +65,17 @@
   else tail[c] = acc;
 }
 
-__global__ void __launch_bounds__(256) k_abc_rows(const uint32_t* __restrict__ rp, size_t n, uint32_t K,
-                                                  const Fr* __restrict__ head, const Fr* __restrict__ tail,
-                                                  Fr* __restrict__ abc) {
-  ZK_WT(WT_ABC_ROWS);
-  ZK_LIGHT();
+template <bool PACKED>
+__global__ void __launch_bounds__(64) k_abc_chunks(const uint32_t* __restrict__ rp, uint32_t nrows, AbcTerms T,
+                                                   const Fr* __restrict__ w, uint32_t K, Fr* __restrict__ head,
+                                                   Fr* __restrict__ tail, Fr* __restrict__ abc) {
+  ZK_WT(WT_ABC);
+  ZK_LIGHT();
+  abc_chunk<PACKED>(rp, nrows, T, w, K, head, tail, abc);
+}
+
+ZK_DEV void abc_rows_lane(const uint32_t* __restrict__ rp, size_t n, uint32_t K, const Fr* __restrict__ head,
+                          const Fr* __restrict__ tail, Fr* __restrict__ abc) {
   const size_t j = (size_t)blockIdx.x * blockDim.x + threadIdx.x;
   if (j >= n) return;
   const Fr a = abc_row(rp, (uint32_t)j, K, head, tail, abc);
@@ -78,6 +83,98 @@
   abc[j] = a;
   abc[n + j] = b;
   abc[2 * n + j] = fp_mul(a, b);
+}
+
+__global__ void __launch_bounds__(256) k_abc_rows(const uint32_t* __restrict__ rp, size_t n, uint32_t K,
+                                                  const Fr* __restrict__ head, const Fr* __restrict__ tail,
+                                                  Fr* __restrict__ abc) {
+  ZK_WT(WT_ABC_ROWS);
+  ZK_LIGHT();
+  abc_rows_lane(rp, n, K, head, tail, abc);
+}
+
+
+template <bool PACKED>
+__global__ void __launch_bounds__(64) k_abc_chunks_when(const uint32_t* __restrict__ rp, uint32_t nrows, AbcTerms T,
+                                                        const Fr* __restrict__ w, uint32_t K, Fr* __restrict__ head,
+                                                        Fr* __restrict__ tail, Fr* __restrict__ abc,
+                                                        const uint32_t* __restrict__ state, uint32_t when) {
+  if ((state[1] != 0) != (when != 0)) return;
+  ZK_WT(WT_ABC);
+  ZK_LIGHT();
+  abc_chunk<PACKED>(rp, nrows, T, w, K, head, tail, abc);
+}
+
+__global__ void __launch_bounds__(256) k_abc_rows_plain(const uint32_t* __restrict__ rp, size_t n, uint32_t K,
+                                                        const Fr* __restrict__ head, const Fr* __restrict__ tail,
+                                                        Fr* __restrict__ abc, const uint32_t* __restrict__ state) {
+  if (!state[1]) return;
+  ZK_WT(WT_ABC_ROWS);
+  ZK_LIGHT();
+  abc_rows_lane(rp, n, K, head, tail, abc);
+}
+
+__global__ void __launch_bounds__(256) k_abc_rows_grouped(const uint32_t* __restrict__ crp,
+                                                          const uint32_t* __restrict__ cls, size_t n, uint32_t Kd,
+                                                          const Fr* __restrict__ head, const Fr* __restrict__ tail,
+                                                          const Fr* __restrict__ cls_val, Fr* __restrict__ abc,
+                                                          const uint32_t* __restrict__ state) {
+  if (state[1]) return;
+  ZK_WT(WT_ABC_ROWS);
+  ZK_LIGHT();
+  const size_t j = (size_t)blockIdx.x * blockDim.x + threadIdx.x;
+  if (j >= n) return;
+  const Fr a = abc_row(crp, cls[j], Kd, head, tail, cls_val);
+  const Fr b = abc_row(crp, cls[n + j], Kd, head, tail, cls_val);
+  abc[j] = a;
+  abc[n + j] = b;
+  abc[2 * n + j] = fp_mul(a, b);
+}
+
+constexpr int FIX_LANES = 8, FIX_T = 256, FIX_BLOCKS_MAX = 256;
+template <bool PACKED>
+__global__ void __launch_bounds__(FIX_T) k_abc_fix(const uint32_t* __restrict__ rp, AbcTerms T,
+                                                   const Fr* __restrict__ w, size_t n,
+                                                   const uint32_t* __restrict__ state,
+                                                   const uint32_t* __restrict__ dirty, uint32_t cap,
+                                                   Fr* __restrict__ abc, uint32_t* __restrict__ report) {
+  if (blockIdx.x == 0 && threadIdx.x == 0) {
+    report[0] = state[0];
+    report[1] = state[1];
+  }
+  if (state[1]) return;
+  ZK_WT(WT_ABC_ROWS);
+  ZK_LIGHT();
+  const uint32_t cnt = state[0] < cap ? state[0] : cap;
+  const uint32_t lane = threadIdx.x % FIX_LANES;
+  const uint32_t cmask = PACKED ? (1u << T.cshift) - 1u : 0xFFFFFFFFu;
+  const uint32_t step = gridDim.x * (FIX_T / FIX_LANES);
+  for (uint32_t d = (blockIdx.x * FIX_T + threadIdx.x) / FIX_LANES; d < cnt; d += step) {
+    const uint32_t j = dirty[d];
+    Fr ab[2];
+#pragma unroll
+    for (int h = 0; h < 2; h++) {
+      const uint32_t r = h ? (uint32_t)n + j : j, e = rp[r + 1];
+      Fr acc = fp_zero<FrP>();
+      for (uint32_t p = rp[r] + lane; p < e; p += FIX_LANES) {
+        const uint32_t t = T.cols[p];
+        acc = fp_add(acc, fp_mul(PACKED ? T.coefs[t >> T.cshift] : T.coefs[p], w[t & cmask]));
+      }
+#pragma unroll
+      for (int off = FIX_LANES / 2; off; off >>= 1) {
+        Fr o;
+#pragma unroll
+        for (int k = 0; k < 8; k++) o.v[k] = __shfl_xor(acc.v[k], off, FIX_LANES);
+        acc = fp_add(acc, o);
+      }
+      ab[h] = acc;
+    }
+    if (lane == 0) {
+      abc[j] = ab[0];
+      abc[n + j] = ab[1];
+      abc[2 * n + j] = fp_mul(ab[0], ab[1]);
+    }
+  }
 }
 
 __global__ void k_join(const Fr* __restrict__ abc, size_t n, Fr* __restrict__ h) {
@@ -107,6 +204,9 @@
     for (size_t i = ((size_t)y * gridDim.x + blockIdx.x) * blockDim.x + threadIdx.x; i < ps.w_nvec; i += nb)
       ps.w_dst[i] = src[i];
   }
+  if (y == 0 && ps.gr_state)
+    for (uint32_t i = blockIdx.x * blockDim.x + threadIdx.x; i < ps.gr_words; i += gridDim.x * blockDim.x)
+      ps.gr_state[i] = 0u;
   if (y == 0 && blockIdx.x == 2 && threadIdx.x < RS_WORDS) d_rs[threadIdx.x] = rs_host[threadIdx.x];
   if (y == 0 && blockIdx.x == 0 && threadIdx.x == 0) {
     const Fr* rs = reinterpret_cast<const Fr*>(rs_host);
@@ -161,6 +261,29 @@
   hipLaunchKernelGGL(k_abc_rows, dim3(zk_grid(n, 256)), dim3(256), 0, st, rp, n, K, head, tail, abc);
 }
 
+void abc_grouped(hipStream_t st, const AbcGrouped& G, const uint32_t* rp, size_t n, const AbcTerms& T, const Fr* w,
+                 uint32_t K, Fr* head, Fr* tail, Fr* abc) {
+  auto chunks = [&](const uint32_t* rows, uint32_t nrows, const AbcTerms& terms, uint32_t k, Fr* whole, uint32_t when) {
+    const dim3 grid(zk_grid((k + ABC_L - 1) / ABC_L, 64));
+    if (terms.cshift)
+      hipLaunchKernelGGL(k_abc_chunks_when<true>, grid, dim3(64), 0, st, rows, nrows, terms, w, k, head, tail, whole,
+                         G.state, when);
+    else
+      hipLaunchKernelGGL(k_abc_chunks_when<false>, grid, dim3(64), 0, st, rows, nrows, terms, w, k, head, tail, whole,
+                         G.state, when);
+  };
+  chunks(G.crp, G.classes, G.terms, G.Kd, G.cls_val, 0);
+  hipLaunchKernelGGL(k_abc_rows_grouped, dim3(zk_grid(n, 256)), dim3(256), 0, st, G.crp, G.cls, n, G.Kd, head, tail,
+                     G.cls_val, abc, G.state);
+  const dim3 fix_grid(std::min<unsigned>(zk_grid((size_t)G.cap * FIX_LANES, FIX_T), FIX_BLOCKS_MAX));
+  if (T.cshift)
+    hipLaunchKernelGGL(k_abc_fix<true>, fix_grid, dim3(FIX_T), 0, st, rp, T, w, n, G.state, G.dirty, G.cap, abc, G.report);
+  else
+    hipLaunchKernelGGL(k_abc_fix<false>, fix_grid, dim3(FIX_T), 0, st, rp, T, w, n, G.state, G.dirty, G.cap, abc, G.report);
+  chunks(rp, (uint32_t)(2 * n), T, K, abc, 1);
+  hipLaunchKernelGGL(k_abc_rows_plain, dim3(zk_grid(n, 256)), dim3(256), 0, st, rp, n, K, head, tail, abc, G.state);
+}
+
 void join_h(hipStream_t st, const Fr* abc, size_t n, Fr* h) {
   hipLaunchKernelGGL(k_join, dim3(zk_grid(n, 256)), dim3(256), 0, st, abc, n, h);
 }
diff --git a/verifiable-federated-training-with-zero-knowledge-proofs-zk-fl-_amd/csrc/prove.hip b/verifiable-federated-training-with-zero-knowledge-proofs-zk-fl-_amd/csrc/prove.hip
--- a/verifiable-federated-training-with-zero-knowledge-proofs-zk-fl-_amd/csrc/prove.hip
+++ b/verifiable-federated-training-with-zero-knowledge-proofs-zk-fl-_amd/csrc/prove.hip
@@ -55,7 +55,7 @@
   msm_scratch_free(s->g2s);
   msm_tail_free(s->g2t);
   void* ptrs[] = {s->abc, s->abc_head, s->abc_tail, s->h, s->res, s->resB2, s->d_rs, s->d_parts,
-                  s->w_stage, s->grp_cnt};
+                  s->w_stage, s->grp_cnt, s->gr_state, s->gr_dirty, s->gr_missing, s->cls_val};
   for (void* p : ptrs)
     if (p) (void)hipFree(p);
   if (s->pinned) (void)hipHostFree(s->pinned);
@@ -113,6 +113,11 @@
   s->extra = s->h + n;
   ZK_CHECK(hipMalloc(&s->grp_cnt, 2 * sizeof(uint32_t)));
   ZK_CHECK(hipMemsetAsync(s->grp_cnt, 0, 2 * sizeof(uint32_t), st));
+  if (may_group && k->ctx->opts.group_rows && k->K && k->logn > k->ctx->opts.small_logn) {
+    ZK_CHECK(hipMalloc(&s->gr_state, group_rows_state_words(n) * sizeof(uint32_t)));
+    ZK_CHECK(hipMalloc(&s->gr_missing, (size_t)group_rows_miss_cap((uint32_t)n) * sizeof(uint32_t)));
+    ZK_CHECK(hipMalloc(&s->gr_dirty, (size_t)group_rows_dirty_cap((uint32_t)n) * sizeof(uint32_t)));
+  }
   s->key = k;
   ZK_CHECK(hipMalloc(&s->abc, n * 3 * 32));
   const size_t abc_chunks = (k->K + ABC_L - 1) / ABC_L + 1;
@@ -263,6 +268,7 @@
   bool fast_wsum;
   bool graph;
   bool grouped;
+  bool group_rows;
 };
 
 struct PlanBases {
@@ -279,6 +285,7 @@
   ProofPlan p = {};
   p.mode = mode;
   p.grouped = mode == ProofMode::Proof && k->grp.on && !ZK_KNOCKOUT;
+  p.group_rows = p.grouped && k->grp.rows_on && s->gr_state;
   const bool plain = mode == ProofMode::Proof && k->share_b && !prof->serialize && !ZK_KNOCKOUT;
   const bool want_lowlat = batch_of_one && o.lowlat;
   p.graph = o.graph && s->w_stage && !want_lowlat && plain && !prof->on && s->direct_proofs > 0;
@@ -320,19 +327,40 @@
     ps.w_dst = reinterpret_cast<uint4*>(s->w_stage);
     ps.w_nvec = (uint32_t)((size_t)k->nVars * 32 / sizeof(uint4));
   }
+  if (p.group_rows) {
+    ps.gr_state = s->gr_state;
+    ps.gr_words = (uint32_t)group_rows_state_words(k->n);
+  }
   proof_start(s->st_main, reinterpret_cast<const uint32_t*>(s->pinned + 256), reinterpret_cast<uint32_t*>(s->d_rs),
               s->extra, parts, res3, ps);
 }
 
-hipError_t abc_ntt(zkfl_key* k, ProofSlot* s, const Fr* d_w, hipStream_t st, Profiler* prof) {
+inline GroupMark group_mark(const zkfl_key* k, const ProofSlot* s, const ProofPlan& p) {
+  if (!p.group_rows) return GroupMark{};
+  return {k->grp.d_wstart, k->grp.d_wlist, s->gr_state, s->gr_missing, group_rows_miss_cap(k->n), s->gr_dirty,
+          group_rows_dirty_cap(k->n)};
+}
+
+void abc_stage(zkfl_key* k, ProofSlot* s, const Fr* d_w, hipStream_t st, const ProofPlan& p) {
+  const size_t n = k->n;
+  const uint32_t K = (uint32_t)k->K;
+  const AbcTerms T = {k->cols, k->coefs, k->cshift};
+  if (p.group_rows) {
+    const KeyGroups& g = k->grp;
+    const AbcTerms R = {g.d_cterms, k->cshift ? k->coefs : g.d_ccoefs, k->cshift};
+    const AbcGrouped G = {g.d_crp, g.row_classes, R, g.terms_rep, g.d_cls, s->cls_val, s->gr_state, s->gr_dirty,
+                          group_rows_dirty_cap(k->n), reinterpret_cast<uint32_t*>(s->pinned + MISS_OFF) + 1};
+    abc_grouped(st, G, k->rows, n, T, d_w, K, s->abc_head, s->abc_tail, s->abc);
+    return;
+  }
+  if (K) abc_chunks(st, k->rows, (uint32_t)(2 * n), T, d_w, K, s->abc_head, s->abc_tail, s->abc);
+  abc_rows(st, k->rows, n, K, s->abc_head, s->abc_tail, s->abc);
+}
+
+hipError_t abc_ntt(zkfl_key* k, ProofSlot* s, const Fr* d_w, hipStream_t st, const ProofPlan& p, Profiler* prof) {
   const size_t n = k->n;
   int pi = prof->begin("abc", st);
-  if (k->K) {
-    const uint32_t K = (uint32_t)k->K;
-    const AbcTerms T = {k->cols, k->coefs, k->cshift};
-    abc_chunks(st, k->rows, (uint32_t)(2 * n), T, d_w, K, s->abc_head, s->abc_tail, s->abc);
-  }
-  abc_rows(st, k->rows, n, (uint32_t)k->K, s->abc_head, s->abc_tail, s->abc);
+  abc_stage(k, s, d_w, st, p);
   prof->end(pi, st, (double)k->K);
   pi = prof->begin("ntt", st);
   if (!(ZK_KNOCKOUT & 4)) ZK_CHECK(ntt_coset_shift(k->ntt, s->abc, 3, n, st));
@@ -388,7 +416,7 @@
   if (k->a_diff) fold_a(sa, s->res);
   assemble_t(sa, s->res, glv_halves(s), proof_out(s));
   HIP_TRY(hipEventRecord(ev_t, sa), "event");
-  HIP_TRY(abc_ntt(k, s, d_w, st, prof), "ntt");
+  HIP_TRY(abc_ntt(k, s, d_w, st, p, prof), "ntt");
   HIP_TRY(msm_accumulate(b.CH, s->g1s, s->g1t[2], W, (const uint32_t*)s->h, st, prof, "msm_accumulate_g1"),
           "msm C+H");
   HIP_TRY(msm_tails(&tails[2], &outs[2], 1, st, p.fast_wsum), "msm tail C+H");
@@ -403,7 +431,7 @@
 int run_front(zkfl_key* k, ProofSlot* s, const Fr* d_w, const ProofPlan& p, Profiler* prof) {
   hipStream_t st = s->st_main;
   const uint32_t *W = (const uint32_t*)d_w, *E = (const uint32_t*)s->extra;
-  HIP_TRY(abc_ntt(k, s, d_w, st, prof), "ntt");
+  HIP_TRY(abc_ntt(k, s, d_w, st, p, prof), "ntt");
   const PlanBases b = plan_bases(k, p);
   const MsmBases<FqOps>* bs[3] = {&b.A, &b.B1, &b.CH};
   MsmScratch<FqOps>* ss[3] = {&s->g1s_a, &s->g1s_b, &s->g1s};
@@ -441,7 +469,7 @@
   G2P* o2 = s->resB2;
   if (!p.share_b_sort && !(ZK_KNOCKOUT & 32))
     HIP_TRY(msm_run(b.B2, s->g2s, s->g2t, W, E, s->resB2, st, prof, "msm_accumulate_g2"), "msm B2");
-  if (p.light_first) HIP_TRY(abc_ntt(k, s, d_w, st, prof), "ntt");
+  if (p.light_first) HIP_TRY(abc_ntt(k, s, d_w, st, p, prof), "ntt");
   HIP_TRY(msm_accumulate(b.A, sA, s->g1t[0], W, E, st, prof, "msm_accumulate_g1"), "msm A");
   if (p.share_b_sort) {
     HIP_TRY(msm_sort(b.B1, sB, s->g1t[1].nnz, W, E, st), "msm B1 sort");
@@ -453,7 +481,7 @@
     HIP_TRY(msm_accumulate(b.B1, sB, s->g1t[1], W, E, st, prof, "msm_accumulate_g1"), "msm B1");
   }
   if (parts) HIP_TRY(msm_accumulate(b.CH, s->g1s, s->g1t[2], W, Z, st, prof, "msm_accumulate_g1"), "msm C");
-  if (!p.light_first) HIP_TRY(abc_ntt(k, s, d_w, st, prof), "ntt");
+  if (!p.light_first) HIP_TRY(abc_ntt(k, s, d_w, st, p, prof), "ntt");
   if (parts)
     HIP_TRY(msm_accumulate(b.CH, s->g1s, s->g1t[3], Z, H, st, prof, "msm_accumulate_g1"), "msm H");
   else
@@ -472,7 +500,8 @@
   start(k, s, p);
   if (p.grouped)
     group_delta(s->st_main, d_w, k->grp.d_rep, k->nVars, s->extra + 4, s->grp_cnt,
-                reinterpret_cast<uint32_t*>(s->pinned + MISS_OFF));
+                reinterpret_cast<uint32_t*>(s->pinned + MISS_OFF), group_mark(k, s, p));
+  if (p.group_rows) group_mark_rows(s->st_main, group_mark(k, s, p));
   const int rc = p.schedule == Schedule::Lowlat  ? run_lowlat(k, s, d_w, p, prof)
                  : p.schedule == Schedule::Front ? run_front(k, s, d_w, p, prof)
                                                  : run_chain(k, s, d_w, p, prof);
@@ -507,6 +536,14 @@
   glv_split(rs_host, ks[2], ks[3]);
   const ProofPlan p = plan_proof(ctx->opts, k, s, mode, batch_of_one, &ctx->prof);
   s->grouped_run = p.grouped;
+  s->rows_run = p.group_rows;
+  if (p.group_rows && s->cls_cap < k->grp.row_classes) {
+    if (s->cls_val) (void)hipFree(s->cls_val);
+    s->cls_val = nullptr;
+    s->cls_cap = 0;
+    HIP_TRY(hipMalloc(&s->cls_val, (size_t)k->grp.row_classes * 32), "class values");
+    s->cls_cap = k->grp.row_classes;
+  }
   int rc;
   if (p.graph) {
     const uint64_t src = reinterpret_cast<uint64_t>(d_w);
@@ -536,7 +573,15 @@
   HIP_TRY(host_wait(s->ev_done, poll), "sync");
   if (s->out_proof) memcpy(s->out_proof, s->pinned, 256);
   if (s->out_part) memcpy(s->out_part, s->pinned + 512, PART_WORDS * 4);
-  if (s->grouped_run) memcpy(&s->key->grp.last_miss, s->pinned + MISS_OFF, 4);
+  if (s->grouped_run) {
+    uint32_t c[3];
+    memcpy(c, s->pinned + MISS_OFF, sizeof(c));
+    KeyGroups& g = s->key->grp;
+    g.last_miss = c[0];
+    g.last_dirty = s->rows_run ? c[1] : 0;
+    g.last_plain = s->rows_run ? c[2] : 0;
+  }
+  s->rows_run = false;
   s->grouped_run = false;
   s->busy = false;
   return ZKFL_OK;
@@ -1078,4 +1123,46 @@
   return rc;
 }
 
-}
+int zkfl_debug_abc(zkfl_ctx* ctx, zkfl_key* key, const zkfl_witness* w, int grouped, uint8_t* abc_out,
+                   uint32_t* counts_out) {
+  if (!ctx || !key || !w || !abc_out || !counts_out) return fail(ZKFL_E_ARG, "debug_abc: null argument");
+  if (key->ctx != ctx) return fail(ZKFL_E_ARG, "debug_abc: key of another context");
+  if (w->key != key) return fail(ZKFL_E_MISMATCH, "witness uploaded for another key");
+  HIP_TRY(hipSetDevice(ctx->device), "hipSetDevice");
+  ProofSlot* s = nullptr;
+  int rc = get_slot(key, 0, &s);
+  if (rc) return rc;
+  if (s->busy && (rc = wait_slot(s))) return rc;
+  ProofPlan p = {};
+  p.mode = ProofMode::Proof;
+  p.grouped = grouped && key->grp.on;
+  p.group_rows = p.grouped && key->grp.rows_on && s->gr_state;
+  p.share_b_sort = key->share_b;
+  if (p.group_rows && s->cls_cap < key->grp.row_classes) {
+    if (s->cls_val) (void)hipFree(s->cls_val);
+    s->cls_val = nullptr;
+    s->cls_cap = 0;
+    HIP_TRY(hipMalloc(&s->cls_val, (size_t)key->grp.row_classes * 32), "class values");
+    s->cls_cap = key->grp.row_classes;
+  }
+  memset(s->pinned + 256, 0, 64 + 4 * sizeof(GlvScalar));
+  memset(s->pinned + MISS_OFF, 0, 12);
+  hipStream_t st = s->st_main;
+  start(key, s, p);
+  if (p.grouped)
+    group_delta(st, w->d, key->grp.d_rep, key->nVars, s->extra + 4, s->grp_cnt,
+                reinterpret_cast<uint32_t*>(s->pinned + MISS_OFF), group_mark(key, s, p));
+  if (p.group_rows) group_mark_rows(st, group_mark(key, s, p));
+  abc_stage(key, s, w->d, st, p);
+  const size_t n3 = 3 * (size_t)key->n;
+  fr_mont_to_std(st, s->abc, n3);
+  hipError_t e = hipGetLastError();
+  if (e == hipSuccess) e = hipMemcpyAsync(abc_out, s->abc, n3 * 32, hipMemcpyDeviceToHost, st);
+  if (e == hipSuccess) e = hipStreamSynchronize(st);
+  if (e != hipSuccess) return hip_fail(e, "debug abc");
+  memcpy(counts_out, s->pinned + MISS_OFF, 12);
+  if (!p.group_rows) counts_out[1] = counts_out[2] = 0;
+  return ZKFL_OK;
+}
+
+}
diff --git a/verifiable-federated-training-with-zero-knowledge-proofs-zk-fl-_amd/csrc/zkfl.hip b/verifiable-federated-training-with-zero-knowledge-proofs-zk-fl-_amd/csrc/zkfl.hip
--- a/verifiable-federated-training-with-zero-knowledge-proofs-zk-fl-_amd/csrc/zkfl.hip
+++ b/verifiable-federated-training-with-zero-knowledge-proofs-zk-fl-_amd/csrc/zkfl.hip
@@ -219,6 +219,8 @@
   ctx->opts.ab_shared = env("ZKFL_AB_SHARED", 1) != 0;
   ctx->opts.groups = env("ZKFL_GROUPS", 1) != 0;
   ctx->opts.group_min_batch = std::max(1, env("ZKFL_GROUP_MIN_BATCH", 8));
+  ctx->opts.group_rows = env("ZKFL_GROUP_ROWS", 1) != 0;
+  ctx->opts.group_rows_cap = std::max(0, env("ZKFL_GROUP_ROWS_CAP", 0));
   hipError_t e = hipStreamCreateWithFlags(&ctx->st, hipStreamNonBlocking);
   if (e != hipSuccess) {
     delete ctx;
diff --git a/verifiable-federated-training-with-zero-knowledge-proofs-zk-fl-_amd/zkfl/native.py b/verifiable-federated-training-with-zero-knowledge-proofs-zk-fl-_amd/zkfl/native.py
--- a/verifiable-federated-training-with-zero-knowledge-proofs-zk-fl-_amd/zkfl/native.py
+++ b/verifiable-federated-training-with-zero-knowledge-proofs-zk-fl-_amd/zkfl/native.py
@@ -58,6 +58,12 @@
     _fields_ = [("grouped", C.c_uint32), ("learned", C.c_uint32), ("groups", C.c_uint32), ("non_rep", C.c_uint32),
                 ("bases", C.c_uint32 * 4), ("bases_rep", C.c_uint32 * 4), ("builds", C.c_uint32),
                 ("last_miss", C.c_uint32), ("build_ms", C.c_double)]
+
+
+class GroupRowsInfo(C.Structure):
+    _fields_ = [("rows_grouped", C.c_uint32), ("row_classes", C.c_uint32), ("terms", C.c_uint32),
+                ("terms_rep", C.c_uint32), ("wire_list", C.c_uint32), ("wires_over_cap", C.c_uint32),
+                ("last_dirty", C.c_uint32), ("last_plain", C.c_uint32), ("rows_build_ms", C.c_double)]
 
 
 SIGNATURES = {
@@ -88,9 +94,14 @@
     "zkfl_key_set_groups": (C.c_int, [_P, C.POINTER(C.c_uint32), C.c_size_t]),
     "zkfl_key_learn_groups": (C.c_int, [_P, _P, _P]),
     "zkfl_key_groups": (C.c_int, [_P, C.POINTER(GroupsInfo)]),
+    "zkfl_key_group_rows": (C.c_int, [_P, C.POINTER(GroupRowsInfo)]),
     "zkfl_debug_groups": (C.c_int, [C.c_char_p, C.c_char_p, C.c_size_t, C.POINTER(C.c_uint32), C.POINTER(C.c_uint32),
                                     C.c_size_t, C.c_uint32, C.POINTER(C.c_uint32), C.POINTER(C.c_uint32),
                                     C.POINTER(C.c_uint32)]),
+    "zkfl_debug_group_rows": (C.c_int, [C.POINTER(C.c_uint32), C.c_uint32, C.POINTER(C.c_uint32), C.c_uint32,
+                                        C.POINTER(C.c_uint32), C.POINTER(C.c_uint32), C.c_uint32, C.c_uint32,
+                                        C.c_uint32] + [C.POINTER(C.c_uint32)] * 7),
+    "zkfl_debug_abc": (C.c_int, [_P, _P, _P, C.c_int, _U8P, C.POINTER(C.c_uint32)]),
     "zkfl_key_set_slots": (C.c_int, [_P, C.c_int]),
     "zkfl_groth16_prove": (C.c_int, [_P, _P, C.c_char_p, C.c_size_t, C.c_char_p, _U8P, _U8P,
                                      C.POINTER(C.c_size_t)]),
@@ -628,9 +639,20 @@
     def groups(self) -> dict:
         g = GroupsInfo()
         check(lib().zkfl_key_groups(self.h, C.byref(g)))
+        r = GroupRowsInfo()
+        check(lib().zkfl_key_group_rows(self.h, C.byref(r)))
         return {"grouped": bool(g.grouped), "learned": bool(g.learned), "groups": g.groups, "non_rep": g.non_rep,
                 "bases": dict(zip(GROUP_QUERIES, g.bases)), "bases_rep": dict(zip(GROUP_QUERIES, g.bases_rep)),
-                "builds": g.builds, "last_miss": g.last_miss, "build_ms": g.build_ms}
+                "builds": g.builds, "last_miss": g.last_miss, "build_ms": g.build_ms,
+                "rows_grouped": bool(r.rows_grouped), "row_classes": r.row_classes, "terms": r.terms,
+                "terms_rep": r.terms_rep, "wire_list": r.wire_list, "wires_over_cap": r.wires_over_cap,
+                "last_dirty": r.last_dirty, "last_plain": bool(r.last_plain), "rows_build_ms": r.rows_build_ms}
+
+    def debug_abc(self, w: "ResidentWitness", grouped: bool = True):
+        out = _buf(96 * self.domain_size)
+        cnt = (C.c_uint32 * 3)()
+        check(lib().zkfl_debug_abc(self.ctx.h, self.h, w.h, 1 if grouped else 0, out, cnt))
+        return bytes(out), cnt[0], cnt[1], bool(cnt[2])
 
     def set_slots(self, slots: int):
         check(lib().zkfl_key_set_slots(self.h, slots))
```

Result: faster. 853.2 proofs/s (median of 6 runs) (+4.7%).
